# themattrosen/Planeverb

Hardware: AMD Instinct MI355X
Metric: grid_cell_updates_per_s (higher is better)
Workload: dtype f32

## Files before the change

### include/planeverb_amd.h

```cpp
#ifndef PLANEVERB_AMD_H
#define PLANEVERB_AMD_H

#include <stddef.h>
#include <stdint.h>

#ifdef __cplusplus
extern "C" {
#endif

#if defined(__GNUC__)
#define PVA_EXPORT __attribute__((visibility("default")))
#else
#define PVA_EXPORT
#endif


typedef struct PlaneverbOutput {
    float occlusion;
    float wetGain;
    float rt60;
    float lowpass;
    float directionX;
    float directionY;
    float sourceDirectionX;
// ... 78 lines not shown
    int tileRows, tileCols;
    int pitch, rows;
    int histRows, histPitch;
    int numGeometry;
    long long deviceBytes;
    int streamFuse;
    int residentKernel;
} PvAmdInfo;

typedef struct PvAmdTimings {
    float fdtdMs;
    float analysisMs;
    float geometryMs;
    float stepKernelMs;
    int stepLaunches;
    float airKernelMs;
    float generalKernelMs;
    int airLaunches, generalLaunches;
    float stepLoopMs;
    int reachedCells;
    int activeCells;
    int silentCells;
} PvAmdTimings;

enum {
    PVA_OPT_DENSE_HISTORY = 1,
    PVA_OPT_NUM_STEPS = 2,
    PVA_OPT_SKIP_ANALYSIS = 3,
    PVA_OPT_USE_GRAPH = 4,
    PVA_OPT_STEPS_PER_LAUNCH = 5,
    PVA_OPT_TILE_ROWS = 6,
    PVA_OPT_NO_FREE_GRID = 7,
    PVA_OPT_TIME_KERNELS = 8,
    PVA_OPT_TILE_ORDER = 9,
    PVA_OPT_SMALL_GRID_KERNEL = 10,
    PVA_OPT_PACKED_MATH = 11,
    PVA_OPT_STREAMING_ANALYSIS = 12,
    PVA_OPT_STREAM_ROWS = 13,
    PVA_OPT_MERGED_LAUNCH = 14,
    PVA_OPT_ROW_BANDS = 16,
    PVA_OPT_PATCH_KERNEL = 17,
    PVA_OPT_LAZY_FAR_CELLS = 19,
    PVA_OPT_STREAM_FUSE = 20,
    PVA_OPT_AUX_STREAMS = 21,
    PVA_OPT_RESIDENT_KERNEL = 22,
    PVA_OPT_RT60_LANES = 23,
    PVA_OPT_FUSED_ANALYSIS = 29,
    PVA_OPT_ANALYSIS_FORK = 28,
    PVA_OPT_STREAM_PRIORITY = 25,
    PVA_OPT_ALTERNATE_SWEEPS = 26,
    PVA_OPT_XCD_REGIONS = 27,
    PVA_OPT_REACH_BOUND = 30,
    PVA_OPT_RESIDENT_WINDOW = 31,
    PVA_OPT_DEBUG_LOSE_FIRST_CAPTURE = 24,
    PVA_OPT_PATCH_STRIP = 18,
    PVA_OPT_EDGE_TILES = 15
};

PVA_EXPORT int PvAmdDeviceCount(void);
PVA_EXPORT const char* PvAmdLastError(void);
PVA_EXPORT const char* PvAmdVersion(void);

PVA_EXPORT PvAmdSolver* PvAmdCreate(float gridSizeX, float gridSizeY, int gridResolution, int device);
PVA_EXPORT PvAmdSolver* PlaneverbCreateGrid(float gridSizeX, float gridSizeY, int gridResolution, int device);
PVA_EXPORT PvAmdSolver* PvAmdCreateSlabs(float gridSizeX, float gridSizeY, int gridResolution, const int* devices,
                                         int nslabs);
typedef struct PvAmdSlabInfo {
    int nslabs;
    int row0[16], rows[16], device[16];
    long long haloBytesPerLaunch;
    long long exchangeBytesPerRun;
    long long deviceBytes[16];
    int handoffWords;
    int streamRedeals;
    float dryRunUsPerSweep;
} PvAmdSlabInfo;
PVA_EXPORT int PvAmdGetSlabInfo(PvAmdSolver* s, PvAmdSlabInfo* out);
PVA_EXPORT PvAmdSolver* PvAmdCreateSlabRank(float gridSizeX, float gridSizeY, int gridResolution, int device,
                                            int slabIndex, int slabCount);
PVA_EXPORT int PvAmdComputeEfree(float gridSizeX, float gridSizeY, int gridResolution, int device, float* efree);
PVA_EXPORT int PvAmdSlabSetEfree(PvAmdSolver* slab, float efree);
PVA_EXPORT int PvAmdSlabBegin(PvAmdSolver* slab, float lx, float ly, float lz);
PVA_EXPORT int PvAmdSlabNumLaunches(PvAmdSolver* slab);
PVA_EXPORT int PvAmdSlabLaunch(PvAmdSolver* slab, int li);
PVA_EXPORT int PvAmdSlabHaloFloats(PvAmdSolver* slab);
PVA_EXPORT int PvAmdSlabExportHalo(PvAmdSolver* slab, int side, float* host);
PVA_EXPORT int PvAmdSlabImportHalo(PvAmdSolver* slab, int side, const float* host);
PVA_EXPORT int PvAmdSlabHistoryFloats(PvAmdSolver* slab);
PVA_EXPORT int PvAmdSlabExportEdgeHistory(PvAmdSolver* slab, float* host);
PVA_EXPORT int PvAmdSlabImportAboveHistory(PvAmdSolver* slab, const float* host);
PVA_EXPORT int PvAmdSlabAnalyze(PvAmdSolver* slab);
PVA_EXPORT long long PvAmdSlabWindowBlock(PvAmdSolver* slab, int* info4, float* host, long long capacityFloats);
typedef struct PvAmdSlabRoot PvAmdSlabRoot;
PVA_EXPORT PvAmdSlabRoot* PvAmdSlabRootCreate(PvAmdSolver* anySlab, int device);
PVA_EXPORT void PvAmdSlabRootDestroy(PvAmdSlabRoot* r);
PVA_EXPORT int PvAmdSlabRootBegin(PvAmdSlabRoot* r, float lx, float ly, float lz);
PVA_EXPORT int PvAmdSlabRootImportBlock(PvAmdSlabRoot* r, const int* info4, const float* host);
PVA_EXPORT int PvAmdSlabRootFinish(PvAmdSlabRoot* r);
PVA_EXPORT int PvAmdSlabRootGetOutput(PvAmdSlabRoot* r, float ex, float ey, float ez, PlaneverbOutput* out);
PVA_EXPORT int PvAmdSlabRootCopyResults(PvAmdSlabRoot* r, float* res8, float* delay);
PVA_EXPORT void PvAmdDestroy(PvAmdSolver* s);
PVA_EXPORT int PvAmdSetOption(PvAmdSolver* s, int key, long long value);
PVA_EXPORT int PvAmdGetInfo(PvAmdSolver* s, PvAmdInfo* out);

PVA_EXPORT int PvAmdAddGeometry(PvAmdSolver* s, float posX, float posY, float width, float height,
                                float absorption);
// ... 2 lines not shown
PVA_EXPORT int PvAmdRemoveGeometry(PvAmdSolver* s, int id);
PVA_EXPORT int PvAmdLoadScene(PvAmdSolver* s, const char* pvPath);
PVA_EXPORT int PvAmdSaveScene(PvAmdSolver* s, const char* pvPath);

PVA_EXPORT int PvAmdAddShape(PvAmdSolver* s, const float* xy, int n, float absorption);
PVA_EXPORT int PvAmdUpdateShape(PvAmdSolver* s, int id, const float* xy, int n, float absorption);
PVA_EXPORT int PvAmdRemoveShape(PvAmdSolver* s, int id);
PVA_EXPORT int PvAmdAddOrientedBox(PvAmdSolver* s, float px, float py, float w, float h, float ax, float ay, float absorption);
PVA_EXPORT int PvAmdUpdateOrientedBox(PvAmdSolver* s, int id, float px, float py, float w, float h, float ax, float ay,
                                      float absorption);
#define PVA_POLY_MAX_VERTS 64
PVA_EXPORT int PvAmdAddDisc(PvAmdSolver* s, float cx, float cy, float radius, float absorption);
PVA_EXPORT int PvAmdUpdateDisc(PvAmdSolver* s, int id, float cx, float cy, float radius, float absorption);
PVA_EXPORT int PvAmdAddCapsule(PvAmdSolver* s, float ax, float ay, float bx, float by, float radius, float absorption);
PVA_EXPORT int PvAmdUpdateCapsule(PvAmdSolver* s, int id, float ax, float ay, float bx, float by, float radius, float absorption);
PVA_EXPORT int PvAmdAddWallPath(PvAmdSolver* s, const float* xy, int n, float radius, float absorption);
PVA_EXPORT int PvAmdUpdateWallPath(PvAmdSolver* s, int id, const float* xy, int n, float radius, float absorption);
PVA_EXPORT int PvAmdAddPolygon(PvAmdSolver* s, const float* xy, int n, float absorption);
PVA_EXPORT int PvAmdUpdatePolygon(PvAmdSolver* s, int id, const float* xy, int n, float absorption);
#define PVA_MESH_SOLID 0
#define PVA_MESH_SHELL 1
#define PVA_MESH_MAX 64
#define PVA_MESH_MAX_TRIS (1 << 20)
#define PVA_MESH_MAX_TRIS_TOTAL (1 << 22)
PVA_EXPORT int PvAmdAddMesh(PvAmdSolver* s, const float* verts, int nv, const int* tris, int nt, float absorption, int mode,
                            float radius);
PVA_EXPORT int PvAmdUpdateMesh(PvAmdSolver* s, int id, const float* verts, int nv, const int* tris, int nt, float absorption,
                               int mode, float radius);
PVA_EXPORT int PvAmdSetMeshTransform(PvAmdSolver* s, int id, const float m12[12]);
PVA_EXPORT int PvAmdRemoveMesh(PvAmdSolver* s, int id);
PVA_EXPORT int PvAmdSetSliceHeight(PvAmdSolver* s, float h);
PVA_EXPORT float PvAmdGetSliceHeight(PvAmdSolver* s);
PVA_EXPORT int PvAmdMeshTriangles(PvAmdSolver* s, int id);
PVA_EXPORT int PvAmdCopyMeshSection(PvAmdSolver* s, int id, float* out4nt, uint8_t* valid_nt);
PVA_EXPORT int PvAmdHostMeshSection(const float* verts, int nv, const int* tris, int nt, const float* m12_or_null, float h,
                                    float* out4nt, uint8_t* valid_nt);
PVA_EXPORT int PvAmdHostMeshCoverage(float gridSizeX, float gridSizeY, int gridResolution, const float* verts, int nv,
                                     const int* tris, int nt, const float* m12_or_null, float h, int mode, float radius,
                                     uint8_t* cover);
PVA_EXPORT int PvAmdSetGridBoundary(PvAmdSolver* s, const float absorption4[4]);
PVA_EXPORT int PvAmdGetGridBoundary(PvAmdSolver* s, float out4[4]);
PVA_EXPORT int PvAmdSetEdgeLayer(PvAmdSolver* s, const int width4[4]);
PVA_EXPORT int PvAmdGetEdgeLayer(PvAmdSolver* s, int out4[4]);
#define PVA_EDGE_LAYER_SPLIT_R0 1e-4
PVA_EXPORT int PvAmdSetEdgeLayerSplit(PvAmdSolver* s, const int width4[4], double r0);
PVA_EXPORT int PvAmdGetEdgeLayerModel(PvAmdSolver* s, int* split, double* r0);
PVA_EXPORT int PvAmdHostEdgeLayerTables(float gridSizeX, float gridSizeY, int gridResolution, const int width4[4], float* out);
PVA_EXPORT int PvAmdHostEdgeLayerTablesR0(float gridSizeX, float gridSizeY, int gridResolution, const int width4[4], double r0,
                                          float* out);
PVA_EXPORT int PvAmdHostEnclosure(const uint8_t* beta, int nx, int ny, int seedX, int seedY, int tileRows, int tileCols, int maxTiles,
                                  int* out10);
PVA_EXPORT int PvAmdHostWindowClear(int windowRun, const int* win4, const int* prevRect4, int planesDirty, int sweptDirty,
                                    int splitPlanes);
PVA_EXPORT int PvAmdHostOrientedBoxVertices(float px, float py, float w, float h, float ax, float ay, float* out8);
PVA_EXPORT int PvAmdHostShape(const float* xy, int n, float absorption, float* out16);
PVA_EXPORT int PvAmdHostShapeCoverage(float gridSizeX, float gridSizeY, int gridResolution, const float* xy, int n,
                                      uint8_t* cover);
#define PVA_SHAPE_DISC 1
#define PVA_SHAPE_CAPSULE 2
#define PVA_SHAPE_WALL_PATH 3
#define PVA_SHAPE_POLYGON 4
PVA_EXPORT int PvAmdHostRoundShapeCoverage(float gridSizeX, float gridSizeY, int gridResolution, int kind, const float* xy,
                                           int n, float radius, uint8_t* cover);

PVA_EXPORT int PvAmdRun(PvAmdSolver* s, float lx, float ly, float lz);
PVA_EXPORT int PvAmdRunAsync(PvAmdSolver* s, float lx, float ly, float lz);
PVA_EXPORT int PvAmdRunAsyncAfter(PvAmdSolver* s, PvAmdSolver* prev, float lx, float ly, float lz);
PVA_EXPORT int PvAmdSync(PvAmdSolver* s);
PVA_EXPORT int PvAmdRunBatch(PvAmdSolver* const* solvers, int n, const float* listenersXYZ, int wait);
PVA_EXPORT float PvAmdClockProbe(int device, float* byMemtimeMHz);
PVA_EXPORT int PvAmdBandwidthProbe(int device, float* gbPerS4);
#define PVA_LIBM_LOG10               0
#define PVA_LIBM_LOG10_NONNEG        1
#define PVA_LIBM_LOG10_NONNEG_TAB    2
#define PVA_LIBM_LOG10_NORMAL_TAB    3
#define PVA_LIBM_LOG10_NORMAL_BATCH  4
#define PVA_LIBM_POW_08              5
#define PVA_LIBM_POW_23              6
#define PVA_LIBM_POW_NONNEG_08       7
#define PVA_LIBM_POW_NONNEG_23       8
#define PVA_LIBM_POW_NONNEG_TAB_08   9
#define PVA_LIBM_POW_NONNEG_TAB_23  10
PVA_EXPORT int PvAmdLibmProbe(int form, const float* in, float* out, long long n, int onDevice);
PVA_EXPORT int PvAmdGetTimings(PvAmdSolver* s, PvAmdTimings* out);
PVA_EXPORT int PvAmdLastRunResidentWindow(PvAmdSolver* s);
PVA_EXPORT int PvAmdLastRunOneXcd(PvAmdSolver* s);

PVA_EXPORT int PvAmdSetEmitters(PvAmdSolver* s, const float* xyz, int n);
PVA_EXPORT int PvAmdGetOutput(PvAmdSolver* s, float ex, float ey, float ez, PlaneverbOutput* out);
PVA_EXPORT int PvAmdSetOutputQueries(PvAmdSolver* s, const float* xyz, int n);
PVA_EXPORT int PvAmdGetQueriedOutputs(PvAmdSolver* s, PlaneverbOutput* out, int n);
#define PVA_QREC_ROOM_METRICS   1u
#define PVA_QREC_DECAY_TIMES    2u
#define PVA_QREC_LATERAL        4u
#define PVA_QREC_ECHOGRAM       8u
#define PVA_QREC_ECHO_CRITERION 16u
#define PVA_QREC_LOBES          32u
PVA_EXPORT int PvAmdSetQueryRecords(PvAmdSolver* s, unsigned kinds);
PVA_EXPORT unsigned PvAmdGetQueryRecordKinds(PvAmdSolver* s);
PVA_EXPORT int PvAmdQueryRecordFloats(PvAmdSolver* s, unsigned kind);
PVA_EXPORT int PvAmdGetQueriedRecords(PvAmdSolver* s, unsigned kind, float* out, int nQueries);
#define PVA_RECORD_QUERIES_MAX 1024
PVA_EXPORT int PvAmdSetRecordQueries(PvAmdSolver* s, const float* xyz, int n);
#define PVA_QSPEC_BAND_METRICS 1u
#define PVA_QSPEC_MODULATION   2u
#define PVA_QSPEC_SPECTRUM     4u
PVA_EXPORT int PvAmdSetQuerySpectralRecords(PvAmdSolver* s, unsigned kinds);
PVA_EXPORT unsigned PvAmdGetQuerySpectralKinds(PvAmdSolver* s);
PVA_EXPORT int PvAmdQuerySpectralFloats(PvAmdSolver* s, unsigned kind);
PVA_EXPORT int PvAmdGetQueriedSpectralRecords(PvAmdSolver* s, unsigned kind, float* out, int nQueries);
PVA_EXPORT int PvAmdSetEmitterRecords(PvAmdSolver* s, unsigned timeKinds, unsigned spectralKinds);
PVA_EXPORT int PvAmdGetEmitterRecordKinds(PvAmdSolver* s, unsigned* timeKinds, unsigned* spectralKinds);
PVA_EXPORT int PvAmdEmitterRecordFloats(PvAmdSolver* s, int family, unsigned kind);
PVA_EXPORT int PvAmdGetEmitterRecords(PvAmdSolver* s, int family, unsigned kind, float* out, int nEmitters);
PVA_EXPORT int PvAmdGetEmitterCells(PvAmdSolver* s, int* cxcy, int cap);
PVA_EXPORT int PvAmdCopyEmitterTrace(PvAmdSolver* s, int emitter, float* outT);
PVA_EXPORT int PvAmdCopyResults(PvAmdSolver* s, float* res8, float* delay);
PVA_EXPORT int PvAmdCopyResultsBlock(PvAmdSolver* s, int r0, int c0, int nr, int nc, float* res8, float* delay);
PVA_EXPORT int PvAmdGetImpulseResponse(PvAmdSolver* s, int cx, int cy, float* out3T);
PVA_EXPORT int PvAmdGetImpulseResponseCells(PvAmdSolver* s, int cx, int cy, PlaneverbCell* outT);
PVA_EXPORT int PvAmdCopyFields(PvAmdSolver* s, float* pr, float* vx, float* vy);
PVA_EXPORT int PvAmdCopyHistoryPlane(PvAmdSolver* s, int t, float* pr);
PVA_EXPORT int PvAmdSetHistoryPlane(PvAmdSolver* s, int t, const float* pr);
typedef struct PvAmdRoomMetrics {
    float c50, c80, d50, ts, e50, l50, e80, l80, total, moment;
} PvAmdRoomMetrics;
PVA_EXPORT int PvAmdComputeRoomMetrics(PvAmdSolver* s, float* ms);
PVA_EXPORT int PvAmdCopyRoomMetrics(PvAmdSolver* s, float* out10);
PVA_EXPORT int PvAmdCopyRoomMetricsBlock(PvAmdSolver* s, int r0, int c0, int nr, int nc, float* out10);
PVA_EXPORT int PvAmdGetRoomMetrics(PvAmdSolver* s, float ex, float ey, float ez, PvAmdRoomMetrics* out);
PVA_EXPORT int PvAmdHostRoomMetrics(const float* p, int T, int fs, int onset, PvAmdRoomMetrics* out);
typedef struct PvAmdDecayTimes {
    float edt, t20, t30, n_edt, n_t20, n_t30, e0, depth;
} PvAmdDecayTimes;
PVA_EXPORT int PvAmdComputeDecayTimes(PvAmdSolver* s, float* ms);
PVA_EXPORT int PvAmdCopyDecayTimes(PvAmdSolver* s, float* out8);
PVA_EXPORT int PvAmdCopyDecayTimesBlock(PvAmdSolver* s, int r0, int c0, int nr, int nc, float* out8);
PVA_EXPORT int PvAmdGetDecayTimes(PvAmdSolver* s, float ex, float ey, float ez, PvAmdDecayTimes* out);
// ... 248 lines not shown
```

### planeverb_amd/api.py

```python
import ctypes as C
import os
from collections import namedtuple

import numpy as np

from .build import LIB_PATH

PV_INVALID_DRY_GAIN = -1.0
PV_INVALID_ID = -1

PVA_OPT_DENSE_HISTORY = 1
PVA_OPT_NUM_STEPS = 2
PVA_OPT_SKIP_ANALYSIS = 3
PVA_OPT_USE_GRAPH = 4
PVA_OPT_STEPS_PER_LAUNCH = 5
PVA_OPT_TILE_ROWS = 6
PVA_OPT_NO_FREE_GRID = 7
PVA_OPT_TIME_KERNELS = 8
PVA_OPT_TILE_ORDER = 9
PVA_OPT_SMALL_GRID_KERNEL = 10
PVA_OPT_PACKED_MATH = 11
PVA_OPT_STREAMING_ANALYSIS = 12
PVA_OPT_STREAM_ROWS = 13
PVA_OPT_MERGED_LAUNCH = 14
PVA_OPT_EDGE_TILES = 15
PVA_OPT_ROW_BANDS = 16
PVA_OPT_PATCH_KERNEL = 17
PVA_OPT_PATCH_STRIP = 18
PVA_OPT_LAZY_FAR_CELLS = 19
PVA_OPT_STREAM_FUSE = 20
PVA_OPT_AUX_STREAMS = 21
PVA_OPT_RESIDENT_KERNEL = 22
PVA_OPT_RT60_LANES = 23
PVA_OPT_DEBUG_LOSE_FIRST_CAPTURE = 24
PVA_OPT_STREAM_PRIORITY = 25
PVA_OPT_ALTERNATE_SWEEPS = 26
PVA_OPT_XCD_REGIONS = 27
PVA_OPT_ANALYSIS_FORK = 28
PVA_OPT_FUSED_ANALYSIS = 29
PVA_OPT_REACH_BOUND = 30
PVA_OPT_RESIDENT_WINDOW = 31


class PlaneverbOutput(C.Structure):
    _fields_ = [("occlusion", C.c_float), ("wetGain", C.c_float), ("rt60", C.c_float), ("lowpass", C.c_float),
                ("directionX", C.c_float), ("directionY", C.c_float), ("sourceDirectionX", C.c_float),
                ("sourceDirectionY", C.c_float)]

    def as_array(self):
        return np.array([self.occlusion, self.wetGain, self.rt60, self.lowpass, self.directionX, self.directionY,
                         self.sourceDirectionX, self.sourceDirectionY], np.float32)


class PlaneverbCell(C.Structure):
    _fields_ = [("pr", C.c_float), ("vx", C.c_float), ("vy", C.c_float), ("b", C.c_short), ("by", C.c_short)]


CELL_DTYPE = np.dtype([("pr", np.float32), ("vx", np.float32), ("vy", np.float32), ("b", np.int16), ("by", np.int16)])


class PvAmdInfo(C.Structure):
    _fields_ = [("gx", C.c_int), ("gy", C.c_int), ("T", C.c_int), ("fs", C.c_int), ("res", C.c_int),
                ("dx", C.c_float), ("dt", C.c_float), ("efree", C.c_float), ("device", C.c_int),
                ("stepsPerLaunch", C.c_int), ("tileRows", C.c_int), ("tileCols", C.c_int), ("pitch", C.c_int),
                ("rows", C.c_int), ("histRows", C.c_int), ("histPitch", C.c_int), ("numGeometry", C.c_int),
                ("deviceBytes", C.c_longlong), ("streamFuse", C.c_int), ("residentKernel", C.c_int)]


class PvAmdBakeInfo(C.Structure):
    _fields_ = [("gx", C.c_int), ("gy", C.c_int), ("T", C.c_int), ("fs", C.c_int), ("res", C.c_int), ("dx", C.c_float),
                ("stride", C.c_int), ("x0", C.c_float), ("z0", C.c_float), ("sx", C.c_float), ("sz", C.c_float),
                ("nx", C.c_int), ("nz", C.c_int), ("probesBaked", C.c_int), ("probesInvalid", C.c_int),
                ("records", C.c_longlong), ("materialHash", C.c_ulonglong)]


class PvAmdSlabInfo(C.Structure):
    _fields_ = [("nslabs", C.c_int), ("row0", C.c_int * 16), ("rows", C.c_int * 16), ("device", C.c_int * 16),
                ("haloBytesPerLaunch", C.c_longlong), ("exchangeBytesPerRun", C.c_longlong),
                ("deviceBytes", C.c_longlong * 16), ("handoffWords", C.c_int), ("streamRedeals", C.c_int),
                ("dryRunUsPerSweep", C.c_float)]


class PvAmdTimings(C.Structure):
    _fields_ = [("fdtdMs", C.c_float), ("analysisMs", C.c_float), ("geometryMs", C.c_float),
                ("stepKernelMs", C.c_float), ("stepLaunches", C.c_int), ("airKernelMs", C.c_float), ("generalKernelMs", C.c_float), ("airLaunches", C.c_int),
                ("generalLaunches", C.c_int), ("stepLoopMs", C.c_float), ("reachedCells", C.c_int), ("activeCells", C.c_int), ("silentCells", C.c_int)]


ROOM_METRIC_NAMES = ("c50", "c80", "d50", "ts", "e50", "l50", "e80", "l80", "total", "moment")


class PvAmdRoomMetrics(C.Structure):
    _fields_ = [(n, C.c_float) for n in ROOM_METRIC_NAMES]

# ... 116 lines not shown
    "PvAmdUpdateGeometry": (C.c_int, [_vp, C.c_int] + [C.c_float] * 5),
    "PvAmdRemoveGeometry": (C.c_int, [_vp, C.c_int]),
    "PvAmdLoadScene": (C.c_int, [_vp, C.c_char_p]),
    "PvAmdSaveScene": (C.c_int, [_vp, C.c_char_p]),
    "PvAmdAddShape": (C.c_int, [_vp, _fp, C.c_int, C.c_float]),
    "PvAmdUpdateShape": (C.c_int, [_vp, C.c_int, _fp, C.c_int, C.c_float]),
    "PvAmdRemoveShape": (C.c_int, [_vp, C.c_int]),
    "PvAmdAddOrientedBox": (C.c_int, [_vp] + [C.c_float] * 7),
    "PvAmdUpdateOrientedBox": (C.c_int, [_vp, C.c_int] + [C.c_float] * 7),
    "PvAmdAddDisc": (C.c_int, [_vp] + [C.c_float] * 4),
    "PvAmdUpdateDisc": (C.c_int, [_vp, C.c_int] + [C.c_float] * 4),
    "PvAmdAddCapsule": (C.c_int, [_vp] + [C.c_float] * 6),
    "PvAmdUpdateCapsule": (C.c_int, [_vp, C.c_int] + [C.c_float] * 6),
    "PvAmdAddWallPath": (C.c_int, [_vp, _fp, C.c_int, C.c_float, C.c_float]),
    "PvAmdUpdateWallPath": (C.c_int, [_vp, C.c_int, _fp, C.c_int, C.c_float, C.c_float]),
    "PvAmdAddPolygon": (C.c_int, [_vp, _fp, C.c_int, C.c_float]),
    "PvAmdUpdatePolygon": (C.c_int, [_vp, C.c_int, _fp, C.c_int, C.c_float]),
    "PvAmdAddMesh": (C.c_int, [_vp, _fp, C.c_int, C.POINTER(C.c_int), C.c_int, C.c_float, C.c_int, C.c_float]),
    "PvAmdUpdateMesh": (C.c_int, [_vp, C.c_int, _fp, C.c_int, C.POINTER(C.c_int), C.c_int, C.c_float, C.c_int, C.c_float]),
    "PvAmdSetMeshTransform": (C.c_int, [_vp, C.c_int, _fp]),
    "PvAmdRemoveMesh": (C.c_int, [_vp, C.c_int]),
    "PvAmdSetSliceHeight": (C.c_int, [_vp, C.c_float]),
    "PvAmdGetSliceHeight": (C.c_float, [_vp]),
    "PvAmdMeshTriangles": (C.c_int, [_vp, C.c_int]),
    "PvAmdCopyMeshSection": (C.c_int, [_vp, C.c_int, _fp, C.POINTER(C.c_ubyte)]),
    "PvAmdHostMeshSection": (C.c_int, [_fp, C.c_int, C.POINTER(C.c_int), C.c_int, _fp, C.c_float, _fp, C.POINTER(C.c_ubyte)]),
    "PvAmdHostMeshCoverage": (C.c_int, [C.c_float, C.c_float, C.c_int, _fp, C.c_int, C.POINTER(C.c_int), C.c_int, _fp, C.c_float,
                                        C.c_int, C.c_float, C.POINTER(C.c_ubyte)]),
    "PvAmdSetGridBoundary": (C.c_int, [_vp, _fp]),
    "PvAmdGetGridBoundary": (C.c_int, [_vp, _fp]),
    "PlaneverbSetGridBoundary": (None, [C.c_float] * 4),
    "PvAmdSetEdgeLayer": (C.c_int, [_vp, C.POINTER(C.c_int)]),
    "PvAmdGetEdgeLayer": (C.c_int, [_vp, C.POINTER(C.c_int)]),
    "PlaneverbSetEdgeLayer": (None, [C.c_int] * 4),
    "PvAmdSetEdgeLayerSplit": (C.c_int, [_vp, C.POINTER(C.c_int), C.c_double]),
    "PvAmdGetEdgeLayerModel": (C.c_int, [_vp, C.POINTER(C.c_int), C.POINTER(C.c_double)]),
    "PlaneverbSetEdgeLayerSplit": (None, [C.c_int] * 4),
    "PvAmdHostEdgeLayerTablesR0": (C.c_int, [C.c_float, C.c_float, C.c_int, C.POINTER(C.c_int), C.c_double, _fp]),
    "PvAmdHostEdgeLayerTables": (C.c_int, [C.c_float, C.c_float, C.c_int, C.POINTER(C.c_int), _fp]),
    "PvAmdHostEnclosure": (C.c_int, [C.POINTER(C.c_ubyte)] + [C.c_int] * 7 + [C.POINTER(C.c_int)]),
    "PvAmdHostOrientedBoxVertices": (C.c_int, [C.c_float] * 6 + [_fp]),
    "PvAmdHostShape": (C.c_int, [_fp, C.c_int, C.c_float, _fp]),
    "PvAmdHostShapeCoverage": (C.c_int, [C.c_float, C.c_float, C.c_int, _fp, C.c_int, C.POINTER(C.c_ubyte)]),
    "PvAmdHostRoundShapeCoverage": (C.c_int, [C.c_float, C.c_float, C.c_int, C.c_int, _fp, C.c_int, C.c_float,
                                              C.POINTER(C.c_ubyte)]),
    "PvAmdRun": (C.c_int, [_vp] + [C.c_float] * 3),
    "PvAmdRunAsync": (C.c_int, [_vp] + [C.c_float] * 3),
    "PvAmdRunAsyncAfter": (C.c_int, [_vp, _vp] + [C.c_float] * 3),
    "PvAmdSync": (C.c_int, [_vp]),
    "PvAmdRunBatch": (C.c_int, [C.POINTER(_vp), C.c_int, _fp, C.c_int]),
    "PvAmdGetTimings": (C.c_int, [_vp, C.POINTER(PvAmdTimings)]),
    "PvAmdLastRunResidentWindow": (C.c_int, [_vp]),
    "PvAmdLastRunOneXcd": (C.c_int, [_vp]),
    "PvAmdHostWindowClear": (C.c_int, [C.c_int, C.POINTER(C.c_int), C.POINTER(C.c_int), C.c_int, C.c_int, C.c_int]),
    "PvAmdClockProbe": (C.c_float, [C.c_int, _fp]),
    "PvAmdBandwidthProbe": (C.c_int, [C.c_int, _fp]),
    "PvAmdSetEmitters": (C.c_int, [_vp, _fp, C.c_int]),
    "PvAmdGetOutput": (C.c_int, [_vp] + [C.c_float] * 3 + [C.POINTER(PlaneverbOutput)]),
    "PvAmdSetOutputQueries": (C.c_int, [_vp, _fp, C.c_int]),
    "PvAmdGetQueriedOutputs": (C.c_int, [_vp, C.POINTER(PlaneverbOutput), C.c_int]),
    "PvAmdSetQueryRecords": (C.c_int, [_vp, C.c_uint]),
    "PvAmdGetQueryRecordKinds": (C.c_uint, [_vp]),
    "PvAmdQueryRecordFloats": (C.c_int, [_vp, C.c_uint]),
    "PvAmdGetQueriedRecords": (C.c_int, [_vp, C.c_uint, _fp, C.c_int]),
    "PvAmdSetRecordQueries": (C.c_int, [_vp, _fp, C.c_int]),
    "PvAmdSetQuerySpectralRecords": (C.c_int, [_vp, C.c_uint]),
    "PvAmdGetQuerySpectralKinds": (C.c_uint, [_vp]),
    "PvAmdQuerySpectralFloats": (C.c_int, [_vp, C.c_uint]),
    "PvAmdGetQueriedSpectralRecords": (C.c_int, [_vp, C.c_uint, _fp, C.c_int]),
    "PvAmdSetEmitterRecords": (C.c_int, [_vp, C.c_uint, C.c_uint]),
    "PvAmdGetEmitterRecordKinds": (C.c_int, [_vp, C.POINTER(C.c_uint), C.POINTER(C.c_uint)]),
    "PvAmdEmitterRecordFloats": (C.c_int, [_vp, C.c_int, C.c_uint]),
    "PvAmdGetEmitterRecords": (C.c_int, [_vp, C.c_int, C.c_uint, _fp, C.c_int]),
    "PvAmdGetEmitterCells": (C.c_int, [_vp, C.POINTER(C.c_int), C.c_int]),
    "PvAmdCopyEmitterTrace": (C.c_int, [_vp, C.c_int, _fp]),
    "PvAmdCopyResults": (C.c_int, [_vp, _fp, _fp]),
    "PvAmdCopyResultsBlock": (C.c_int, [_vp, C.c_int, C.c_int, C.c_int, C.c_int, _fp, _fp]),
    "PvAmdGetImpulseResponse": (C.c_int, [_vp, C.c_int, C.c_int, _fp]),
    "PvAmdGetImpulseResponseCells": (C.c_int, [_vp, C.c_int, C.c_int, C.POINTER(PlaneverbCell)]),
    "PvAmdCopyFields": (C.c_int, [_vp, _fp, _fp, _fp]),
    "PvAmdCopyHistoryPlane": (C.c_int, [_vp, C.c_int, _fp]),
    "PvAmdSetHistoryPlane": (C.c_int, [_vp, C.c_int, _fp]),
    "PvAmdLibmProbe": (C.c_int, [C.c_int, _fp, _fp, C.c_longlong, C.c_int]),
    "PvAmdComputeRoomMetrics": (C.c_int, [_vp, _fp]),
    "PvAmdCopyRoomMetrics": (C.c_int, [_vp, _fp]),
    "PvAmdCopyRoomMetricsBlock": (C.c_int, [_vp, C.c_int, C.c_int, C.c_int, C.c_int, _fp]),
    "PvAmdGetRoomMetrics": (C.c_int, [_vp] + [C.c_float] * 3 + [C.POINTER(PvAmdRoomMetrics)]),
    "PvAmdHostRoomMetrics": (C.c_int, [_fp, C.c_int, C.c_int, C.c_int, C.POINTER(PvAmdRoomMetrics)]),
    "PvAmdComputeDecayTimes": (C.c_int, [_vp, _fp]),
    "PvAmdCopyDecayTimes": (C.c_int, [_vp, _fp]),
    "PvAmdCopyDecayTimesBlock": (C.c_int, [_vp, C.c_int, C.c_int, C.c_int, C.c_int, _fp]),
    "PvAmdGetDecayTimes": (C.c_int, [_vp] + [C.c_float] * 3 + [C.POINTER(PvAmdDecayTimes)]),
    "PvAmdHostDecayTimes": (C.c_int, [_fp, C.c_int, C.c_int, C.c_int, C.POINTER(PvAmdDecayTimes)]),
    "PvAmdComputeEchoCriterion": (C.c_int, [_vp, _fp]),
    "PvAmdCopyEchoCriterion": (C.c_int, [_vp, _fp]),
    "PvAmdCopyEchoCriterionBlock": (C.c_int, [_vp, C.c_int, C.c_int, C.c_int, C.c_int, _fp]),
    "PvAmdGetEchoCriterion": (C.c_int, [_vp] + [C.c_float] * 3 + [C.POINTER(PvAmdEchoCriterion)]),
    "PvAmdHostEchoCriterion": (C.c_int, [_fp, C.c_int, C.c_int, C.c_int, C.POINTER(PvAmdEchoCriterion)]),
    "PvAmdComputeLateralFraction": (C.c_int, [_vp, _fp]),
    "PvAmdCopyLateralFraction": (C.c_int, [_vp, _fp]),
    "PvAmdCopyLateralFractionBlock": (C.c_int, [_vp, C.c_int, C.c_int, C.c_int, C.c_int, _fp]),
    "PvAmdGetLateralFraction": (C.c_int, [_vp] + [C.c_float] * 3 + [C.POINTER(PvAmdLateralFraction)]),
    "PvAmdHostLateralFraction": (C.c_int, [_fp, _fp, _fp, C.c_int, C.c_int, C.c_int, C.POINTER(PvAmdLateralFraction)]),
    "PvAmdSetEchogram": (C.c_int, [_vp, C.c_float, C.c_int]),
    "PvAmdGetEchogramSlots": (C.c_int, [_vp, _fp, C.POINTER(C.c_int)]),
    "PvAmdComputeEchogram": (C.c_int, [_vp, _fp]),
# ... 501 lines not shown
    a, n = _xy(vertices)
    cover = np.empty((i.gx + 1, i.gy + 1), np.uint8)
    _check(lib().PvAmdHostShapeCoverage(float(size_x), float(size_y), int(res), _f(a), n,
                                        cover.ctypes.data_as(C.POINTER(C.c_ubyte))))
    return cover


EDGE_LAYER_DEFAULT_WIDTH = 24
EDGE_LAYER_SPLIT_R0 = 1e-4


def _w4(w4):
    a = np.ascontiguousarray(w4, np.int32).reshape(-1)
    if a.size != 4:
        raise ValueError("four widths: x = 0, x = gx, y = 0, y = gy")
    return a


def edge_layer_tables(size_x, size_y, res, w4, r0=None):
    i = host_grid_info(size_x, size_y, res)
    a = _w4(w4)
    out = np.empty(4 * (i.gx + 1) + 4 * (i.gy + 1), np.float32)
    wp = a.ctypes.data_as(C.POINTER(C.c_int))
    if r0 is None:
        n = lib().PvAmdHostEdgeLayerTables(float(size_x), float(size_y), int(res), wp, _f(out))
    else:
        n = lib().PvAmdHostEdgeLayerTablesR0(float(size_x), float(size_y), int(res), wp, float(r0), _f(out))
    if n < 0:
        raise PlaneverbError(last_error())
    nx, ny = i.gx + 1, i.gy + 1
    names = ["apx", "bpx", "ax", "bx", "apy", "bpy", "ay", "by"]
    offs = [0, nx, 2 * nx, 3 * nx, 4 * nx, 4 * nx + ny, 4 * nx + 2 * ny, 4 * nx + 3 * ny]
    return {k: out[o:o + (nx if j < 4 else ny)].copy() for j, (k, o) in enumerate(zip(names, offs))}


def host_enclosure(beta, seed, tile_rows=36, tile_cols=40, max_tiles=128):
    b = np.ascontiguousarray(beta, np.uint8)
    out = np.zeros(10, np.int32)
    if lib().PvAmdHostEnclosure(b.ctypes.data_as(C.POINTER(C.c_ubyte)), b.shape[0], b.shape[1], int(seed[0]), int(seed[1]),
                                int(tile_rows), int(tile_cols), int(max_tiles), out.ctypes.data_as(C.POINTER(C.c_int))) < 0:
        raise PlaneverbError(last_error())
    v = [int(x) for x in out]
    return dict(found=v[0], cells=v[1], box=tuple(v[2:6]), window=tuple(v[6:10]))


def host_window_clear(window_run, win, prev_rect, planes_dirty, swept_dirty, split_planes):
    w, p = ((C.c_int * 4)(*[int(v) for v in r]) for r in (win, prev_rect))
    rc = lib().PvAmdHostWindowClear(int(bool(window_run)), w, p, int(bool(planes_dirty)), int(bool(swept_dirty)), int(bool(split_planes)))
    if rc < 0:
        raise PlaneverbError(last_error())
    return rc


def load_pv(path, max_boxes=4096):
    buf = np.empty((max_boxes, 5), np.float32)
    n = lib().PvAmdHostLoadPv(path.encode(), _f(buf), max_boxes)
    if n < 0:
        raise PlaneverbError(last_error())
    return buf[:n].copy()


def save_pv(path, boxes, ids=None):
    b = np.ascontiguousarray(boxes, np.float32).reshape(-1, 5)
    ida = None if ids is None else np.ascontiguousarray(ids, np.int32)
    _check(lib().PvAmdHostSavePv(path.encode(), _f(b), None if ida is None else ida.ctypes.data_as(C.POINTER(C.c_int)),
                                 len(b)))


def host_room_metrics(p, fs, onset):
    a = np.ascontiguousarray(p, np.float32).reshape(-1)
    out = PvAmdRoomMetrics()
    _check(lib().PvAmdHostRoomMetrics(_f(a) if a.size else None, int(a.size), int(fs), int(onset), out))
    return out.as_array()


def host_decay_times(p, fs, onset):
    a = np.ascontiguousarray(p, np.float32).reshape(-1)
    out = PvAmdDecayTimes()
    _check(lib().PvAmdHostDecayTimes(_f(a) if a.size else None, int(a.size), int(fs), int(onset), out))
    return out.as_array()


def host_echo_criterion(p, fs, onset):
    a = np.ascontiguousarray(p, np.float32).reshape(-1)
    out = PvAmdEchoCriterion()
    _check(lib().PvAmdHostEchoCriterion(_f(a) if a.size else None, int(a.size), int(fs), int(onset), out))
    return out.as_array()


def host_lateral_fraction(p, vx, vy, fs, onset):
    a, x, y = (np.ascontiguousarray(v, np.float32).reshape(-1) for v in (p, vx, vy))
    if not (a.size == x.size == y.size):
        raise ValueError("host_lateral_fraction: p, vx and vy must have the same length")
    out = PvAmdLateralFraction()
    ptr = [_f(v) if v.size else None for v in (a, x, y)]
    _check(lib().PvAmdHostLateralFraction(ptr[0], ptr[1], ptr[2], int(a.size), int(fs), int(onset), out))
    return out.as_array()


ECHOGRAM_MAX_SLOTS = 32


def host_echogram(p, vx, vy, fs, onset, slot_seconds, n_slots):
    a, x, y = (np.ascontiguousarray(v, np.float32).reshape(-1) for v in (p, vx, vy))
    if not (a.size == x.size == y.size):
        raise ValueError("host_echogram: p, vx and vy must have the same length")
# ... 682 lines not shown
    def import_block(self, info4, data):
        info = (C.c_int * 4)(*[int(v) for v in info4])
        data = np.ascontiguousarray(data, np.float32)
        _check(lib().PvAmdSlabRootImportBlock(self._h, info, _f(data) if data.size else None))

    def finish(self):
        _check(lib().PvAmdSlabRootFinish(self._h))

    def get_output(self, emitter):
        o = PlaneverbOutput()
        _check(lib().PvAmdSlabRootGetOutput(self._h, *[float(v) for v in emitter], o))
        return o

    def results(self):
        res = np.empty((self.gx, self.gy, 8), np.float32)
        delay = np.empty((self.gx, self.gy), np.float32)
        _check(lib().PvAmdSlabRootCopyResults(self._h, _f(res), _f(delay)))
        return res, delay


def run_batch(solvers, listeners, wait=True):
    n = len(solvers)
    if n != len(listeners):
        raise ValueError("one listener position per solver")
    hs = (_vp * n)(*[sv._h for sv in solvers])
    xyz = (C.c_float * (3 * n))(*[float(v) for L in listeners for v in L])
    _check(lib().PvAmdRunBatch(hs, n, xyz, 1 if wait else 0))


class Solver:

    def __init__(self, size_x, size_y, res, device=0, slabs=None, **options):
        if slabs is not None:
            dev = (C.c_int * len(slabs))(*[int(d) for d in slabs])
            self._h = lib().PvAmdCreateSlabs(float(size_x), float(size_y), int(res), dev, len(slabs))
        else:
            self._h = lib().PvAmdCreate(float(size_x), float(size_y), int(res), int(device))
        if not self._h:
            raise PlaneverbError(last_error())
        keys = {"dense_history": PVA_OPT_DENSE_HISTORY, "num_steps": PVA_OPT_NUM_STEPS,
                "skip_analysis": PVA_OPT_SKIP_ANALYSIS, "use_graph": PVA_OPT_USE_GRAPH,
                "steps_per_launch": PVA_OPT_STEPS_PER_LAUNCH, "tile_rows": PVA_OPT_TILE_ROWS,
                "no_free_grid": PVA_OPT_NO_FREE_GRID, "time_kernels": PVA_OPT_TIME_KERNELS,
                "tile_order": PVA_OPT_TILE_ORDER, "small_grid_kernel": PVA_OPT_SMALL_GRID_KERNEL,
                "packed_math": PVA_OPT_PACKED_MATH, "streaming_analysis": PVA_OPT_STREAMING_ANALYSIS,
                "stream_rows": PVA_OPT_STREAM_ROWS, "merged_launch": PVA_OPT_MERGED_LAUNCH,
                "edge_tiles": PVA_OPT_EDGE_TILES, "row_bands": PVA_OPT_ROW_BANDS,
                "patch_kernel": PVA_OPT_PATCH_KERNEL, "patch_strip": PVA_OPT_PATCH_STRIP,
                "lazy_far_cells": PVA_OPT_LAZY_FAR_CELLS, "stream_fuse": PVA_OPT_STREAM_FUSE, "aux_streams": PVA_OPT_AUX_STREAMS,
                "resident_kernel": PVA_OPT_RESIDENT_KERNEL, "rt60_lanes": PVA_OPT_RT60_LANES,
                "debug_lose_first_capture": PVA_OPT_DEBUG_LOSE_FIRST_CAPTURE, "stream_priority": PVA_OPT_STREAM_PRIORITY,
                "alternate_sweeps": PVA_OPT_ALTERNATE_SWEEPS, "xcd_regions": PVA_OPT_XCD_REGIONS,
                "analysis_fork": PVA_OPT_ANALYSIS_FORK, "fused_analysis": PVA_OPT_FUSED_ANALYSIS,
                "reach_bound": PVA_OPT_REACH_BOUND, "resident_window": PVA_OPT_RESIDENT_WINDOW}
        for k, v in options.items():
            _check(lib().PvAmdSetOption(self._h, keys[k], int(v)))
        self.info = PvAmdInfo()
        _check(lib().PvAmdGetInfo(self._h, self.info))
        i = self.info
        self.gx, self.gy, self.T, self.fs, self.dx, self.dt, self.efree = i.gx, i.gy, i.T, i.fs, i.dx, i.dt, i.efree
        self._pulse_len = host_grid_info(size_x, size_y, res).T

    def close(self):
        if getattr(self, "_h", None):
            lib().PvAmdDestroy(self._h)
            self._h = None

    def __del__(self):
        try:
            self.close()
        except Exception:
            pass

    def __enter__(self):
        return self

    def __exit__(self, *a):
        self.close()

    def slab_info(self):
        i = PvAmdSlabInfo()
        _check(lib().PvAmdGetSlabInfo(self._h, i))
        return i

    def load_scene(self, path):
        n = lib().PvAmdLoadScene(self._h, path.encode())
        if n < 0:
            raise PlaneverbError(last_error())
        return n

    def save_scene(self, path):
        _check(lib().PvAmdSaveScene(self._h, path.encode()))

    def add_geometry(self, aabb):
        return lib().PvAmdAddGeometry(self._h, *[float(v) for v in aabb])

    def update_geometry(self, gid, aabb):
        _check(lib().PvAmdUpdateGeometry(self._h, int(gid), *[float(v) for v in aabb]))

    def remove_geometry(self, gid):
        _check(lib().PvAmdRemoveGeometry(self._h, int(gid)))

    def add_shape(self, vertices, absorption):
        a, n = _xy(vertices)
        sid = lib().PvAmdAddShape(self._h, _f(a), n, float(absorption))
        if sid < 0:
            raise PlaneverbError(last_error())
# ... 85 lines not shown
        return seg, valid

    def set_grid_boundary(self, r4):
        a = np.ascontiguousarray(r4, np.float32).reshape(-1)
        if a.size != 4:
            raise ValueError("four absorption values: x = 0, x = gx, y = 0, y = gy")
        _check(lib().PvAmdSetGridBoundary(self._h, _f(a)))

    def grid_boundary(self):
        out = np.zeros(4, np.float32)
        _check(lib().PvAmdGetGridBoundary(self._h, _f(out)))
        return out

    def set_edge_layer(self, w4):
        a = _w4(w4)
        _check(lib().PvAmdSetEdgeLayer(self._h, a.ctypes.data_as(C.POINTER(C.c_int))))
        _check(lib().PvAmdGetInfo(self._h, self.info))

    def edge_layer(self):
        out = np.zeros(4, np.int32)
        _check(lib().PvAmdGetEdgeLayer(self._h, out.ctypes.data_as(C.POINTER(C.c_int))))
        return out

    def set_edge_layer_split(self, w4, r0=EDGE_LAYER_SPLIT_R0):
        a = _w4(w4)
        _check(lib().PvAmdSetEdgeLayerSplit(self._h, a.ctypes.data_as(C.POINTER(C.c_int)), float(r0)))
        _check(lib().PvAmdGetInfo(self._h, self.info))

    def edge_layer_model(self):
        sp, r0 = C.c_int(0), C.c_double(0.0)
        _check(lib().PvAmdGetEdgeLayerModel(self._h, C.byref(sp), C.byref(r0)))
        return ("split" if sp.value else "unsplit"), r0.value

    def run(self, listener):
        _check(lib().PvAmdRun(self._h, *[float(v) for v in listener]))

    def run_async(self, listener):
        _check(lib().PvAmdRunAsync(self._h, *[float(v) for v in listener]))

    def run_async_after(self, prev, listener):
        _check(lib().PvAmdRunAsyncAfter(self._h, prev._h, *[float(v) for v in listener]))

    def sync(self):
        _check(lib().PvAmdSync(self._h))

    def run_steps(self, nsteps, with_pulse=False, listener=(0.0, 0.0, 0.0)):
        _check(lib().PvAmdRunSteps(self._h, int(nsteps), int(with_pulse), float(listener[0]), float(listener[2])))

    def last_run_resident_window(self):
        rc = lib().PvAmdLastRunResidentWindow(self._h)
        if rc < 0:
            raise PlaneverbError(last_error())
        return rc == 1

    def last_run_one_xcd(self):
        rc = lib().PvAmdLastRunOneXcd(self._h)
        if rc < 0:
            raise PlaneverbError(last_error())
        return rc == 1

    def timings(self):
        t = PvAmdTimings()
        _check(lib().PvAmdGetTimings(self._h, t))
        return t

    def set_emitters(self, emitters):
        e = np.ascontiguousarray(emitters, np.float32).reshape(-1, 3)
        _check(lib().PvAmdSetEmitters(self._h, _f(e), len(e)))

    def get_output(self, emitter):
        o = PlaneverbOutput()
        _check(lib().PvAmdGetOutput(self._h, *[float(v) for v in emitter], o))
        return o

    def set_output_queries(self, emitters):
        e = np.ascontiguousarray(np.asarray(emitters, np.float32).reshape(-1, 3))
        self._nq = len(e)
        _check(lib().PvAmdSetOutputQueries(self._h, _f(e), len(e)))

    def queried_outputs(self):
        n = getattr(self, "_nq", 0)
        out = (PlaneverbOutput * max(n, 1))()
        _check(lib().PvAmdGetQueriedOutputs(self._h, out, n))
        return np.frombuffer(out, np.float32).reshape(-1, 8)[:n].copy()

    def set_query_records(self, kinds):
        _check(lib().PvAmdSetQueryRecords(self._h, int(kinds)))

    def _record_floats(self, floats, kind):
        n = floats(self._h, int(kind))
        if n < 0:
            raise PlaneverbError(last_error())
        return n

    def _read_records(self, read, kind, shape):
        n = getattr(self, "_nrq", 0) or getattr(self, "_nq", 0)
        out = np.empty((n,) + shape, np.float32)
        _check(read(self._h, int(kind), _f(out) if n else None, n))
        return out

    def query_record_kinds(self):
        return int(lib().PvAmdGetQueryRecordKinds(self._h))

    def query_record_floats(self, kind):
        return self._record_floats(lib().PvAmdQueryRecordFloats, kind)

# ... 570 lines not shown
```

### planeverb_amd/csrc/pv_analysis.h

```cpp
#pragma once

#include <hip/hip_runtime.h>

#include <cfloat>

#include "pv_device.h"
#include "pv_prims.h"

namespace pva {

__device__ __forceinline__ bool analysisAborted(const AnalyzeArgs& a) { return a.abortWord && *a.abortWord != 0u; }

struct NearBox {
    int r0, c0, r1, c1;
    __device__ __forceinline__ bool holds(int r, int c) const { return r >= r0 && r <= r1 && c >= c0 && c <= c1; }
};
__device__ __forceinline__ NearBox nearBoxOf(const int* box, int wr0, int wc0, int wnr, int wnc) {
    NearBox b;
    b.r0 = max(box[0] - 1, wr0);
    b.c0 = max(box[1] - 1, wc0);
    b.r1 = min(box[2] + 1, wr0 + wnr - 1);
    b.c1 = min(box[3] + 1, wc0 + wnc - 1);
    return b;
}
__device__ __forceinline__ NearBox nearBoxOf(const AnalyzeArgs& a, const DynParams& dyn) {
    const int wr0 = dyn.histRow0 - a.G, wc0 = dyn.histCol0 - a.G;
    return nearBoxOf(a.box, wr0, wc0, min(a.winRows, a.gx - wr0), min(a.winCols, a.gy - wc0));
}

__device__ __forceinline__ void farDirectionOf(const FarInfo& f, long long cell, float* ox, float* oy) {
    const int r = (int)(cell / f.gy), c = (int)(cell - (long long)r * f.gy);
    float x = (float)r * f.dx - f.lx, y = (float)c * f.dx - f.lz;
    float len = (x * x) + (y * y);
    if (len != 0.f) {
        len = sqrtf(len);
        x /= len;
        y /= len;
    }
    *ox = x;
    *oy = y;
}
__device__ __forceinline__ bool isFarCell(const FarInfo& f, long long cell) {
    if (!f.on) return false;
    const int r = (int)(cell / f.gy), c = (int)(cell - (long long)r * f.gy);
    if (f.box) return !nearBoxOf(f.box, f.r0, f.c0, f.nr, f.nc).holds(r, c);
    return r < f.r0 || r >= f.r0 + f.nr || c < f.c0 || c >= f.c0 + f.nc;
}

struct CellHistory {
    const float* h;
    long long plane;
    __device__ __forceinline__ float at(int t) const { return h[(long long)t * plane]; }
};

struct PlaneCell {
    bool inGrid;
    int X, Y;
    int tile;
    int row, col;
    int g;
    int hti, htj;
};
__device__ __forceinline__ PlaneCell planeCell(const AnalyzeArgs& a, const DynParams& dyn, long long g) {
    PlaneCell c{false, 0, 0, 0, 0, 0, 0, 0, 0};
// ... 79 lines not shown
```

### planeverb_amd/csrc/pv_analysis.hip

```cpp
#include <hip/hip_runtime.h>

#include <cfloat>
#include <climits>
#include <cstdint>

#include "pv_analysis.h"
#include "pv_analysis_dev.h"
#include "pv_device.h"
#include "pv_launch.h"
#include "pv_libm.h"
#include "pv_prims.h"
#include "pv_record_lane.h"
#include "pv_zone_maps.h"

namespace pva {



template <int CH>
__device__ __forceinline__ void rt60Chunk(const float (&pc)[CH], const int i0, const int startingPoint, float& edc,
                                          float& xysum, float& ysum) {
    float e[CH], y[CH];
#pragma unroll
    for (int k = 0; k < CH; ++k) {
        edc = (i0 - k >= startingPoint) ? edc + pc[k] * pc[k] : edc;
        e[k] = edc;
    }
#pragma unroll
    for (int k = 0; k < CH; ++k) y[k] = 10.f * pvLog10fNonNeg(e[k]);
#pragma unroll
    for (int k = 0; k < CH; ++k) {
        const bool v = i0 - k >= startingPoint;
        xysum = v ? xysum + y[k] * (float)(i0 - k - startingPoint) : xysum;
        ysum = v ? ysum + y[k] : ysum;
    }
}

__device__ __forceinline__ bool analysisWindowCell(const AnalyzeArgs& a, const DynParams& dyn, int* X, int* Y) {
    const int wc = blockIdx.x * blockDim.x + threadIdx.x, wr = blockIdx.y;
    if (wc >= a.winCols) return false;
    *X = dyn.histRow0 - a.G + wr;
    *Y = dyn.histCol0 - a.G + wc;
    return *X < a.gx && *Y < a.gy;
}

#ifndef PV_ONSET_WAVES
#define PV_ONSET_WAVES 4
#endif
#ifndef PV_ONSET_SC
#define PV_ONSET_SC 32
#endif
constexpr int kOnsetWaves = PV_ONSET_WAVES, kOnsetSC = PV_ONSET_SC;
__global__ __launch_bounds__(64 * kOnsetWaves) void pv_onset_kernel(const AnalyzeArgs a) {
    __shared__ int found[64];
    if (analysisAborted(a)) return;
    const DynParams dyn = *a.dyn;
    const int lane = threadIdx.x & 63, wave = __builtin_amdgcn_readfirstlane((int)(threadIdx.x >> 6));
    const long long g = (long long)blockIdx.x * 64 + lane;
    const PlaneCell c = planeCell(a, dyn, g);
    const int T = a.T;
    int tF = INT_MAX;
    bool live = c.inGrid;
    if (live) {
        tF = a.tileFirst[c.tile];
        live = tF < T && a.coef[(size_t)(c.X + a.G) * a.pitch + (c.Y + a.G)].beta != 0.f;
    }
    const bool air = live;
    if (a.labels) {
        const int lX = dyn.lrow - a.G, lY = dyn.lcol - a.G;
        const int mine = live ? a.labels[(size_t)c.X * a.labelNY + c.Y] : -1;
        const int theirs = (lX >= 0 && lX <= a.gx && lY >= 0 && lY < a.labelNY) ? a.labels[(size_t)lX * a.labelNY + lY] : -2;
        live = live && mine == theirs;
    }
    if (wave == 0) found[lane] = INT_MAX;
    if (a.stamp && blockIdx.x == 0 && threadIdx.x == 0) a.stamp[1] = wall_clock64();
    __syncthreads();
    bool inPrev = false;
    if (a.box) {
        const int p0 = a.prevBox[0], p1 = a.prevBox[1], p2 = min(a.prevBox[2], a.gx - 1), p3 = min(a.prevBox[3], a.gy - 1);
        inPrev = c.inGrid && c.X >= p0 && c.X <= p2 && c.Y >= p1 && c.Y <= p3;
        if (p2 >= p0 && p3 >= p1) {
            const int wr0 = dyn.histRow0 - a.G, wc0 = dyn.histCol0 - a.G;
            const int wr1 = wr0 + min(a.winRows, a.gx - wr0) - 1, wc1 = wc0 + min(a.winCols, a.gy - wc0) - 1;
            if (p0 < wr0 || p2 > wr1 || p1 < wc0 || p3 > wc1)
                for (int r = p0 + (int)blockIdx.x; r <= p2; r += (int)gridDim.x)
                    for (int cc = p1 + (int)threadIdx.x; cc <= p3; cc += (int)blockDim.x)
                        if (r < wr0 || r > wr1 || cc < wc0 || cc > wc1) a.delay[r * a.gy + cc] = FLT_MAX;
        }
    }
    if (a.wholeWindow || a.box) {
        if (wave == 0 && c.inGrid && !live && (a.wholeWindow || inPrev)) a.delay[c.X * a.gy + c.Y] = FLT_MAX;
        if (blockIdx.x == 0 && wave == 1) {
            int n = 0;
            for (int i = lane; i < dyn.histTilesX * dyn.histTilesY; i += 64) {
                const int ti = dyn.histTileX0 + i / dyn.histTilesY, tj = dyn.histTileY0 + i % dyn.histTilesY;
                if (a.tileFirst[ti * a.nty + tj] < T) n += a.rxi * a.wi;
            }
#pragma unroll
            for (int off = 1; off < 64; off <<= 1) n += __shfl_xor(n, off);
            if (lane == 0) a.activeCount[0] = n;
        }
    }
    if (__ballot(live) == 0ull) {
        const unsigned long long ms = __ballot(air);
        if (wave == 0 && lane == 0 && ms) atomicAdd(a.activeCount + 3, __popcll(ms));
        return;
    }
    const int m = abs(c.X - (dyn.lrow - a.G)) + abs(c.Y - (dyn.lcol - a.G));
    const int tS = live ? min(max(tF, m), T) : INT_MAX;
    int tBeg = tS;
#pragma unroll
    for (int off = 1; off < 64; off <<= 1) tBeg = min(tBeg, __shfl_xor(tBeg, off));
    tBeg = __builtin_amdgcn_readfirstlane(tBeg);
    const int voff = (int)g * 4;
    const int planeBytes = (int)(a.histPlane * 4);
    constexpr int SC = kOnsetSC;
#pragma unroll 1
    for (int t = tBeg + wave * SC; t < T; t += kOnsetWaves * SC) {
        const int best = found[lane];
        if (__ballot(live && best > t) == 0ull) break;
        float pc[SC];
#pragma unroll
        for (int k = 0; k < SC; ++k) {
            const int tt = t + k;
            const bool want = live && tt >= tS && tt < T && tt < best;
            pc[k] = bufLoadF(makeRsrc(a.hist + (long long)min(tt, T - 1) * a.histPlane, planeBytes), want ? voff : 0x7fffffff, 0);
        }
        int hit = INT_MAX;
#pragma unroll
        for (int k = SC - 1; k >= 0; --k) hit = fabsf(pc[k]) > kAudibleThresholdDev ? t + k : hit;
        if (hit != INT_MAX) atomicMin(&found[lane], hit);
    }
    __syncthreads();
    if (wave != 0) return;
    const int onset = found[lane];
    if (live) {
        if (onset != INT_MAX) a.delay[c.X * a.gy + c.Y] = (float)onset;
        else if (a.wholeWindow || inPrev) a.delay[c.X * a.gy + c.Y] = FLT_MAX;
    }
    const bool reached = live && onset != INT_MAX;
    const unsigned long long mr = __ballot(reached), ms = __ballot(air && !reached);
    if (a.box && mr) {
        int r0 = reached ? c.X : INT_MAX, c0 = reached ? c.Y : INT_MAX, r1 = reached ? c.X : -1, c1 = reached ? c.Y : -1;
#pragma unroll
        for (int off = 1; off < 64; off <<= 1) {
            r0 = min(r0, __shfl_xor(r0, off));
            c0 = min(c0, __shfl_xor(c0, off));
            r1 = max(r1, __shfl_xor(r1, off));
            c1 = max(c1, __shfl_xor(c1, off));
        }
        if (lane == 0) {
            const int b0 = __hip_atomic_load(a.box + 0, __ATOMIC_RELAXED, __HIP_MEMORY_SCOPE_AGENT);
            const int b1 = __hip_atomic_load(a.box + 1, __ATOMIC_RELAXED, __HIP_MEMORY_SCOPE_AGENT);
            const int b2 = __hip_atomic_load(a.box + 2, __ATOMIC_RELAXED, __HIP_MEMORY_SCOPE_AGENT);
            const int b3 = __hip_atomic_load(a.box + 3, __ATOMIC_RELAXED, __HIP_MEMORY_SCOPE_AGENT);
            if (r0 < b0) atomicMin(a.box + 0, r0);
            if (c0 < b1) atomicMin(a.box + 1, c0);
            if (r1 > b2) atomicMax(a.box + 2, r1);
            if (c1 > b3) atomicMax(a.box + 3, c1);
        }
    }
    if (lane == 0) {
        if (mr) {
            atomicAdd(a.activeCount + 1, __popcll(mr));
            a.unitList[atomicAdd(a.activeCount + 4, 1)] = (int)blockIdx.x;
        }
        if (ms) atomicAdd(a.activeCount + 3, __popcll(ms));
    }
}

__global__ __launch_bounds__(256) void pv_encode_kernel(const AnalyzeArgs a) {
    if (analysisAborted(a)) return;
    const DynParams dyn = *a.dyn;
    const int unit = blockIdx.x * 4 + (int)(threadIdx.x >> 6);
    if (unit >= a.activeCount[4]) return;
    const PlaneCell pc0 = planeCell(a, dyn, (long long)a.unitList[unit] * 64 + (threadIdx.x & 63));
    const float delay = pc0.inGrid ? a.delay[pc0.X * a.gy + pc0.Y] : FLT_MAX;
    const bool live = delay != FLT_MAX;
    if (__ballot(live) == 0ull) return;
    encodeWave<false>(a, dyn, pc0, live, live ? (int)delay : 0, rt60LanesPerCell(a, a.activeCount[1]) == 1);
}

template <int L>
__global__ __launch_bounds__(256) void pv_encode_groups_kernel(const AnalyzeArgs a) {
    if (analysisAborted(a)) return;
    const DynParams dyn = *a.dyn;
    constexpr int BPU = L / 4;
    const int unit = blockIdx.x / BPU;
    if (unit >= a.activeCount[4]) return;
    const int ww = (blockIdx.x % BPU) * 4 + (int)(threadIdx.x >> 6), lane = threadIdx.x & 63;
    const PlaneCell pc0 = planeCell(a, dyn, (long long)a.unitList[unit] * 64 + ww * (64 / L) + lane / L);
    const float delay = pc0.inGrid ? a.delay[pc0.X * a.gy + pc0.Y] : FLT_MAX;
    const bool live = delay != FLT_MAX;
    if (__ballot(live) == 0ull) return;
    encodeGroups<L, false>(a, dyn, pc0, lane % L, live, live ? (int)delay : 0);
}

__device__ __forceinline__ void countActiveCells(const AnalyzeArgs& a) {
    __shared__ int part[256];
    const DynParams dyn = *a.dyn;
    int n = 0;
    for (int i = threadIdx.x; i < dyn.histTilesX * dyn.histTilesY; i += 256) {
        const int ti = dyn.histTileX0 + i / dyn.histTilesY, tj = dyn.histTileY0 + i % dyn.histTilesY;
        if (a.tileFirst[ti * a.nty + tj] < a.T) n += a.rxi * a.wi;
    }
    part[threadIdx.x] = n;
    __syncthreads();
    for (int w = 128; w > 0; w >>= 1) {
        if ((int)threadIdx.x < w) part[threadIdx.x] += part[threadIdx.x + w];
        __syncthreads();
    }
    if (threadIdx.x == 0) {
        a.activeCount[0] = part[0];
        a.activeCount[1] = 0;
        a.activeCount[3] = 0;
        a.activeCount[4] = 0;
    }
}
// ... 59 lines not shown
    const float thresholdDist = 0.3f * wavelength;

    while (delay > kDelayCloseDev && loudness < kDistanceGainDev) {
        const int r = cur / a.gy, c = cur - r * a.gy;
        float bestLoud = 0.f, bestDelay = FLT_MAX;
        for (int i = 0; i < 8; ++i) {
            const int nr = r + neighbourDr(i), nc = c + neighbourDc(i);
            if (nr < 0 || nc < 0 || nr >= a.gx || nc >= a.gy) continue;
            const int ni = nr * a.gy + nc;
            const float occ = a.out[ni];
            const float d = a.delay[ni];
            if (occ == 0.f) continue;
            if (d < bestDelay && occ > 0.f) {
                bestLoud = occ;
                cur = ni;
                bestDelay = d;
            }
        }
        if (bestDelay == FLT_MAX || bestDelay >= delay) break;
        delay = bestDelay;
        loudness = bestLoud;
        const float geodesic = kCDev * bestDelay / samplingRate;
        const int r2 = cur / a.gy, c2 = cur - r2 * a.gy;
        const float tx = (float)r2 * a.dx - a.lx, ty = (float)c2 * a.dx - a.lz;
        const float euclid = sqrtf((tx * tx) + (ty * ty));
        if (fabsf(geodesic - euclid) < thresholdDist) break;
    }
    storeDirection(a, index, cur);
}
__global__ __launch_bounds__(256) void pv_direction_kernel(const AnalyzeArgs a) {
    if (analysisAborted(a)) return;
    const DynParams dyn = *a.dyn;
    forDirectionCells(a, dyn, [&](const int index) { directionWalkCell(a, index); });
}

__global__ __launch_bounds__(256) void pv_dir_init_kernel(const AnalyzeArgs a, int* J) {
    if (analysisAborted(a)) return;
    const DynParams dyn = *a.dyn;
    forDirectionCells(a, dyn, [&](const int p) { dirInitCell<false>(a, dyn, J, p); });
}

__global__ __launch_bounds__(256) void pv_dir_jump_kernel(const AnalyzeArgs a, int* J) {
    if (analysisAborted(a)) return;
    const DynParams dyn = *a.dyn;
    forDirectionCells(a, dyn, [&](const int p) { dirJumpCell<false>(a, dyn, J, p); });
}

__global__ __launch_bounds__(256) void pv_dir_final_kernel(const AnalyzeArgs a, const int* J) {
    if (analysisAborted(a)) return;
    const DynParams dyn = *a.dyn;
    forDirectionCells(a, dyn, [&](const int p) { dirFinalCell<false>(a, dyn, J, p); });
}

static dim3 analysisWindowGrid(const AnalyzeArgs& a) { return dim3((a.winCols + 255) / 256, a.winRows); }

static void launchDirectionJump(const AnalyzeArgs& a, int* J, hipStream_t stream) {
    const dim3 grid = analysisWindowGrid(a), block(256);
    hipLaunchKernelGGL(pv_dir_init_kernel, grid, block, 0, stream, a, J);
    for (int i = 0; i < dirJumpPasses(a.T); ++i) hipLaunchKernelGGL(pv_dir_jump_kernel, grid, block, 0, stream, a, J);
    hipLaunchKernelGGL(pv_dir_final_kernel, grid, block, 0, stream, a, J);
}

__global__ void pv_fill_delay_kernel(float* delay, int n) {
    const int i = blockIdx.x * blockDim.x + threadIdx.x;
    if (i < n) delay[i] = FLT_MAX;
}

void launchFarCells(const AnalyzeArgs& a, hipStream_t stream) {
    const int n = a.gx * a.gy;
    hipLaunchKernelGGL(pv_far_cells_kernel, dim3((n + 255) / 256), dim3(256), 0, stream, a);
}

void launchOnset(const AnalyzeArgs& a, hipStream_t stream) {
    hipLaunchKernelGGL(pv_onset_kernel, dim3((unsigned)((a.histPlane + 63) / 64)), dim3(64 * kOnsetWaves), 0, stream, a);
}
void launchEncode(const AnalyzeArgs& a, hipStream_t stream) {
    const unsigned units = (unsigned)((a.histPlane + 63) / 64);
    if (a.rt60Lanes != 1 && a.histPlane <= 16384)
        hipLaunchKernelGGL(pv_encode_groups_kernel<16>, dim3(units * 4), dim3(256), 0, stream, a);
    else if (a.rt60Lanes != 1 && a.histPlane <= kRt60TileMinCells)
        hipLaunchKernelGGL(pv_encode_groups_kernel<4>, dim3(units), dim3(256), 0, stream, a);
    else
        hipLaunchKernelGGL(pv_encode_kernel, dim3((unsigned)((a.histPlane + 255) / 256)), dim3(256), 0, stream, a);
}
void launchRt60(const AnalyzeArgs& a, hipStream_t stream) { launchRt60Forms(a, stream); }

void launchAnalysisCells(const AnalyzeArgs& a, hipStream_t stream) {
    launchOnset(a, stream);
    launchEncode(a, stream);
    launchRt60(a, stream);
}

void launchAnalysisDirection(const AnalyzeArgs& a, hipStream_t stream) {
    const dim3 grid = analysisWindowGrid(a);
    if (a.dirJump)
        launchDirectionJump(a, a.dirScratch, stream);
    else
        hipLaunchKernelGGL(pv_direction_kernel, grid, dim3(256), 0, stream, a);
}

void launchFillDelay(float* delay, long long n, hipStream_t stream) {
    hipLaunchKernelGGL(pv_fill_delay_kernel, dim3((unsigned)((n + 255) / 256)), dim3(256), 0, stream, delay, (int)n);
}

void launchAnalysisFar(const AnalyzeArgs& a, hipStream_t stream) {
    if (a.wholeWindow || a.box) return;
    const int n = a.gx * a.gy;
    if (a.lazyFar) {
        const int nr = max(a.prevNR, min(a.winRows, a.gx)), nc = max(a.prevNC, min(a.winCols, a.gy));
        hipLaunchKernelGGL(pv_far_frame_kernel, dim3((unsigned)((max(nc, 1) + 255) / 256), (unsigned)max(nr, 1), 2), dim3(256), 0,
                           stream, a);
    } else {
        hipLaunchKernelGGL(pv_far_cells_kernel, dim3((n + 255) / 256), dim3(256), 0, stream, a);
    }
}

void launchAnalysis(const AnalyzeArgs& a, hipStream_t stream) {
    launchAnalysisFar(a, stream);
    launchAnalysisCells(a, stream);
    launchAnalysisDirection(a, stream);
}


__global__ __launch_bounds__(256) void pv_stream_accum_kernel(const AnalyzeArgs a) {
    int X, Y;
    if (a.ringList) {
        const int chunks = (a.rxi * a.wi + 255) / 256;
        const int entry = blockIdx.x / chunks;
        const int t = a.ringList[entry];
        const int idx = (blockIdx.x - entry * chunks) * blockDim.x + threadIdx.x;
        if (idx >= a.rxi * a.wi) return;
        const int ti = t / a.nty, r = idx / a.wi;
        X = ti * a.rxi + r;
        Y = (t - ti * a.nty) * a.wi + (idx - r * a.wi);
    } else {
        Y = blockIdx.x * blockDim.x + threadIdx.x;
// ... 227 lines not shown
```

### planeverb_amd/csrc/pv_capi.cpp

```cpp
#include <algorithm>
#include <climits>
#include <cmath>
#include <cstdio>
#include <cstring>
#include <memory>
#include <new>
#include <string>

#include "../../include/planeverb_amd.h"
#include "pv_context.h"
#include "pv_core.h"
#include "pv_bands.h"
#include "pv_modulation.h"
#include "pv_decay.h"
#include "pv_echo.h"
#include "pv_echogram.h"
#include "pv_lateral.h"
#include "pv_lobes.h"
#include "pv_metrics.h"
#include "pv_query_records.h"
#include "pv_query_spectral.h"
#include "pv_spectrum.h"
#include "pv_waterfall.h"
#include "pv_arrays.h"
// ... 640 lines not shown
    std::memset(out, 0, sizeof(*out));
    if (valid)
        std::memcpy(out, v, sizeof(*out));
    else
        out->occlusion = kInvalidDryGain;
    return 0;
} PV_API_CATCH(-1)
int PvAmdSlabRootCopyResults(PvAmdSlabRoot* h, float* res8, float* delay) try {
    return (h && h->r) ? rootRet(h, h->r->copyResults(res8, delay)) : -1;
} PV_API_CATCH(-1)

void PvAmdDestroy(PvAmdSolver* h) try {
    delete h;
} PV_API_CATCH_VOID

int PvAmdSetOption(PvAmdSolver* h, int key, long long value) try {
    if (!h) return -1;
    if (h->s || h->g) {
        g_lastError = "options must be set before the solver is first used";
        return -1;
    }
    switch (key) {
        case PVA_OPT_DENSE_HISTORY: h->opt.denseHistory = value != 0; break;
        case PVA_OPT_NUM_STEPS: h->opt.numSteps = (int)value; break;
        case PVA_OPT_SKIP_ANALYSIS: h->opt.skipAnalysis = value != 0; break;
        case PVA_OPT_USE_GRAPH: h->opt.useGraph = (int)value; break;
        case PVA_OPT_STEPS_PER_LAUNCH: h->opt.K = (int)value; break;
        case PVA_OPT_TILE_ROWS: h->opt.rxi = (int)value; break;
        case PVA_OPT_NO_FREE_GRID: h->opt.withFreeGrid = value == 0; break;
        case PVA_OPT_TIME_KERNELS: h->opt.timeKernels = (int)value; break;
        case PVA_OPT_TILE_ORDER: h->opt.tileOrder = (int)value; break;
        case PVA_OPT_SMALL_GRID_KERNEL: h->opt.smallGrid = (int)value; break;
        case PVA_OPT_PACKED_MATH: h->opt.packed = value != 0; break;
        case PVA_OPT_STREAMING_ANALYSIS: h->opt.streaming = value != 0; break;
        case PVA_OPT_STREAM_ROWS: h->opt.segments = (int)value; break;
        case PVA_OPT_MERGED_LAUNCH: h->opt.merged = (int)value; break;
        case PVA_OPT_EDGE_TILES: h->opt.edgeTiles = value != 0; break;
        case PVA_OPT_ROW_BANDS: h->opt.rowBands = (int)value; break;
        case PVA_OPT_PATCH_KERNEL: h->opt.patch = (int)value; break;
        case PVA_OPT_LAZY_FAR_CELLS: h->opt.lazyFar = value != 0; break;
        case PVA_OPT_STREAM_FUSE: h->opt.streamFuse = (int)value; break;
        case PVA_OPT_AUX_STREAMS: h->opt.auxStreams = (int)std::max<long long>(0, std::min<long long>(value, 8)); break;
        case PVA_OPT_PATCH_STRIP: h->opt.patchStrip = (int)value; break;
        case PVA_OPT_RESIDENT_KERNEL: h->opt.resident = (int)value; break;
        case PVA_OPT_RT60_LANES: h->opt.rt60Lanes = (int)value; break;
        case PVA_OPT_ANALYSIS_FORK: h->opt.analysisFork = (int)value; break;
        case PVA_OPT_FUSED_ANALYSIS: h->opt.fusedAnalysis = (int)value; break;
        case PVA_OPT_DEBUG_LOSE_FIRST_CAPTURE: h->opt.debugLoseFirstCapture = value != 0; break;
        case PVA_OPT_STREAM_PRIORITY: h->opt.streamPriority = (int)value; break;
        case PVA_OPT_ALTERNATE_SWEEPS: h->opt.alternateSweeps = (int)value; break;
        case PVA_OPT_XCD_REGIONS: h->opt.xcdRegions = (int)value; break;
        case PVA_OPT_REACH_BOUND: h->opt.reachBound = (int)value; break;
        case PVA_OPT_RESIDENT_WINDOW: h->opt.residentWindow = (int)value; break;
        default: g_lastError = "unknown option"; return -1;
    }
    return 0;
} PV_API_CATCH(-1)

int PvAmdGetInfo(PvAmdSolver* h, PvAmdInfo* out) try {
    if (!out || !ensure(h, true)) return -1;
    if (h->g) {
        const GridSpec& g = h->g->spec();
        const Solver* s0 = h->g->slab(0);
        std::memset(out, 0, sizeof(*out));
        out->gx = g.gx;
        out->gy = g.gy;
        out->T = h->g->T();
        out->fs = (int)g.fs;
        out->res = g.res;
        out->dx = g.dx;
        out->dt = g.dt;
        out->efree = h->g->efree();
        out->device = s0->device();
        out->stepsPerLaunch = s0->K();
        out->tileRows = s0->geometry().rxi;
        out->tileCols = s0->geometry().wi;
        out->pitch = s0->geometry().pitch;
        out->rows = s0->geometry().rows;
        out->histRows = s0->histRows();
        out->histPitch = s0->histPitch();
        out->numGeometry = h->g->numBoxes();
        out->deviceBytes = h->g->deviceBytes();
        return 0;
    }
    const GridSpec& g = h->s->spec();
    const Geometry& geo = h->s->geometry();
    std::memset(out, 0, sizeof(*out));
    out->gx = g.gx;
    out->gy = g.gy;
    out->T = h->s->T();
    out->fs = (int)g.fs;
    out->res = g.res;
    out->dx = g.dx;
    out->dt = g.dt;
    out->efree = h->s->efree();
    out->device = h->s->device();
    out->stepsPerLaunch = h->s->K();
    out->tileRows = geo.rxi;
    out->tileCols = geo.wi;
    out->pitch = geo.pitch;
    out->rows = geo.rows;
    out->histRows = h->s->histRows();
    out->histPitch = h->s->histPitch();
    out->numGeometry = h->s->numBoxes();
    out->deviceBytes = h->s->deviceBytes();
    out->streamFuse = h->s->streamFuse() ? 1 : 0;
// ... 306 lines not shown
    Solver* s[kBatchMax];
    for (int i = 0; i < n; ++i) {
        if (!wholeGrid(hs[i]) || !ensure(hs[i])) return -1;
        s[i] = hs[i]->s;
    }
    std::string err;
    if (Solver::runBatch(s, n, listenersXYZ, wait != 0, &err)) return 0;
    g_lastError = err.empty() ? "batched run failed" : err;
    return -1;
} PV_API_CATCH(-1)

int PvAmdSync(PvAmdSolver* h) try {
    if (!wholeGrid(h) || !ensure(h)) return -1;
    return ret(h, h->s->sync());
} PV_API_CATCH(-1)

float PvAmdClockProbe(int device, float* byMemtimeMHz) try {
    return clockProbeMHz(device, byMemtimeMHz);
} PV_API_CATCH(0.f)

int PvAmdBandwidthProbe(int device, float* gbPerS4) try {
    if (!gbPerS4) return -1;
    if (bandwidthProbeGBs(device, gbPerS4)) return 0;
    g_lastError = "PvAmdBandwidthProbe: allocation or launch failed (2 GiB of device memory are needed)";
    return -1;
} PV_API_CATCH(-1)

int PvAmdLibmProbe(int form, const float* in, float* out, long long n, int onDevice) try {
    return libmProbe(form, in, out, n, onDevice != 0, &g_lastError) ? 0 : -1;
} PV_API_CATCH(-1)

int PvAmdGetTimings(PvAmdSolver* h, PvAmdTimings* out) try {
    if (!out || !ensure(h, true)) return -1;
    const SolverTimings& t = h->g ? h->g->timings() : h->s->timings();
    out->fdtdMs = t.fdtdMs;
    out->analysisMs = t.analysisMs;
    out->geometryMs = t.geometryMs;
    out->stepLaunches = t.stepLaunches;
    out->stepKernelMs = t.stepLaunches ? t.fdtdMs / (float)t.stepLaunches : 0.f;
    out->airKernelMs = t.airKernelMs;
    out->generalKernelMs = t.generalKernelMs;
    out->airLaunches = t.airLaunches;
    out->generalLaunches = t.generalLaunches;
    out->stepLoopMs = t.stepLoopMs;
    out->reachedCells = t.reachedCells;
    out->activeCells = t.activeCells;
    out->silentCells = t.silentCells;
    return 0;
} PV_API_CATCH(-1)

int PvAmdLastRunResidentWindow(PvAmdSolver* h) try {
    if (!wholeGrid(h) || !ensure(h, true)) return -1;
    return h->s->lastRunResidentWindow() ? 1 : 0;
} PV_API_CATCH(-1)

int PvAmdLastRunOneXcd(PvAmdSolver* h) try {
    if (!wholeGrid(h) || !ensure(h, true)) return -1;
    return h->s->lastRunOneXcd() ? 1 : 0;
} PV_API_CATCH(-1)

int PvAmdSetEmitters(PvAmdSolver* h, const float* xyz, int n) try {
    if (!wholeGrid(h) || !ensure(h) || (n > 0 && !xyz)) return -1;
    return ret(h, h->s->setEmitters(xyz, n));
} PV_API_CATCH(-1)

int PvAmdGetOutput(PvAmdSolver* h, float ex, float ey, float ez, PlaneverbOutput* out) try {
    if (!wholeGrid(h) || !out || !ensure(h, true)) return -1;
    float v[8];
    bool valid = false;
    if (!(h->g ? h->g->getOutput(ex, ey, ez, v, &valid) : h->s->getOutput(ex, ey, ez, v, &valid))) return ret(h, false);
    if (!valid) {
        std::memset(out, 0, sizeof(*out));
        out->occlusion = kInvalidDryGain;
        return 0;
    }
    std::memcpy(out, v, sizeof(*out));
    return 0;
} PV_API_CATCH(-1)

int PvAmdSetOutputQueries(PvAmdSolver* h, const float* xyz, int n) try {
    if (!wholeGrid(h) || (n > 0 && !xyz) || !ensure(h)) return -1;
    return ret(h, h->s->setOutputQueries(xyz, n));
} PV_API_CATCH(-1)

int PvAmdGetQueriedOutputs(PvAmdSolver* h, PlaneverbOutput* out, int n) try {
    if (n < 0 || n > Solver::kMaxQueries || (n > 0 && !out) || !wholeGrid(h) || !ensure(h)) return -1;
    float v[Solver::kMaxQueries * 8];
    unsigned char valid[Solver::kMaxQueries];
    if (!h->s->queriedOutputs(v, valid, n)) return ret(h, false);
    for (int i = 0; i < n; ++i) {
        if (valid[i]) {
            std::memcpy(&out[i], v + 8 * i, sizeof(PlaneverbOutput));
        } else {
            std::memset(&out[i], 0, sizeof(PlaneverbOutput));
            out[i].occlusion = kInvalidDryGain;
        }
    }
    return 0;
} PV_API_CATCH(-1)

static bool analysisHandle(PvAmdSolver* h, const char* pre);
static bool analysisCall(PvAmdSolver* h, const char* pre, const char* fn, const void* out);
static const char kQrecPre[] = "query records: ", kQspecPre[] = "spectral records: ";
static_assert(PVA_QSPEC_BAND_METRICS == 1u << kQspecBandMetrics && PVA_QSPEC_MODULATION == 1u << kQspecModulation &&
                  PVA_QSPEC_SPECTRUM == 1u << kQspecSpectrum,
              "planeverb_amd.h vs pv_query_spectral.h");
// ... 999 lines not shown
} PV_API_CATCH(-1)

static int hostEdgeLayerTables(float sx, float sy, int res, const int* width4, double r0, float* out, const char* name) {
    if (res < kLowResolution || !width4 || !out) {
        g_lastError = std::string(name) + ": resolution below 275 or a null array";
        return -1;
    }
    if (!edgeLayerR0Ok(r0)) {
        g_lastError = std::string(name) + ": r0 must lie strictly between 0 and 1";
        return -1;
    }
    const GridSpec g = makeGridSpec(sx, sy, res);
    if (g.gx < 1 || g.gy < 1) {
        g_lastError = std::string(name) + ": grid has no cells";
        return -1;
    }
    const char* why = edgeLayerRefusal(g.gx, g.gy, width4);
    if (*why) {
        g_lastError = std::string(name) + ": " + why;
        return -1;
    }
    edgeLayerTables(g.gx, g.gy, g.courant, width4, out, r0);
    return 4 * (g.NX + g.NY);
}

int PvAmdHostEdgeLayerTables(float sx, float sy, int res, const int* width4, float* out) try {
    return hostEdgeLayerTables(sx, sy, res, width4, kEdgeLayerR0, out, "PvAmdHostEdgeLayerTables");
} PV_API_CATCH(-1)

int PvAmdHostEdgeLayerTablesR0(float sx, float sy, int res, const int* width4, double r0, float* out) try {
    return hostEdgeLayerTables(sx, sy, res, width4, r0, out, "PvAmdHostEdgeLayerTablesR0");
} PV_API_CATCH(-1)

int PvAmdHostEnclosure(const uint8_t* beta, int nx, int ny, int seedX, int seedY, int tileRows, int tileCols, int maxTiles,
                       int* out10) try {
    if (!beta || !out10 || nx < 1 || ny < 1 || tileRows < 1 || tileCols < 1 || (long long)nx * ny > INT_MAX) {
        g_lastError = "PvAmdHostEnclosure: bad arguments";
        return -1;
    }
    const Enclosure e = findEnclosure(beta, nx, ny, seedX, seedY, tileRows, tileCols, maxTiles, nullptr);
    const int v[10] = {e.found, e.cells, e.r0, e.c0, e.r1, e.c1, e.ti0, e.tj0, e.tis, e.tjs};
    std::copy(v, v + 10, out10);
    return e.cells;
} PV_API_CATCH(-1)

int PvAmdHostWindowClear(int windowRun, const int* win4, const int* prevRect4, int planesDirty, int sweptDirty, int splitPlanes) try {
    if (!win4 || !prevRect4) {
        g_lastError = "PvAmdHostWindowClear: bad arguments";
        return -1;
    }
    return (int)planClear(windowRun != 0, win4, prevRect4, planesDirty != 0, sweptDirty != 0, splitPlanes != 0);
} PV_API_CATCH(-1)

int PvAmdHostLoadPv(const char* path, float* b5, int maxBoxes) try {
    if (!path) return -1;
    std::vector<Box> boxes;
    if (!loadPv(path, &boxes, &g_lastError)) return -1;
    for (int i = 0; i < (int)boxes.size() && i < maxBoxes; ++i) {
        b5[5 * i] = boxes[(size_t)i].x;
        b5[5 * i + 1] = boxes[(size_t)i].y;
        b5[5 * i + 2] = boxes[(size_t)i].w;
        b5[5 * i + 3] = boxes[(size_t)i].h;
        b5[5 * i + 4] = boxes[(size_t)i].R;
    }
    return (int)boxes.size();
} PV_API_CATCH(-1)

int PvAmdHostSavePv(const char* path, const float* b5, const int* ids, int n) try {
    if (!path || (n > 0 && !b5)) return -1;
    std::vector<std::pair<int, Box>> boxes;
    for (int i = 0; i < n; ++i)
        boxes.emplace_back(ids ? ids[i] : i, Box{b5[5 * i], b5[5 * i + 1], b5[5 * i + 2], b5[5 * i + 3], b5[5 * i + 4]});
    return savePv(path, boxes, &g_lastError) ? 0 : -1;
} PV_API_CATCH(-1)

int PvAmdHostRoomMetrics(const float* p, int T, int fs, int onset, PvAmdRoomMetrics* out) try {
    if (!p || !out || T <= 0 || onset < 0 || onset >= T) {
        g_lastError = "PvAmdHostRoomMetrics: an impulse response p[T], T > 0, 0 <= onset < T and an output record";
        return -1;
    }
    static_assert(sizeof(PvAmdRoomMetrics) == kRoomMetricFloats * sizeof(float), "ten floats");
    float v[kRoomMetricFloats];
    roomMetricsOfIr(p, T, fs, onset, v);
    std::memcpy(out, v, sizeof(*out));
    return 0;
} PV_API_CATCH(-1)

int PvAmdHostDecayTimes(const float* p, int T, int fs, int onset, PvAmdDecayTimes* out) try {
    if (!p || !out || T <= 0 || onset < 0 || onset >= T) {
        g_lastError = "decay times: PvAmdHostDecayTimes: an impulse response p[T], T > 0, 0 <= onset < T and an output record";
        return -1;
    }
    static_assert(sizeof(PvAmdDecayTimes) == kDecayFloats * sizeof(float), "eight floats");
    float v[kDecayFloats];
    decayTimesOfIr(p, T, fs, onset, v);
    std::memcpy(out, v, sizeof(*out));
    return 0;
} PV_API_CATCH(-1)

int PvAmdHostLateralFraction(const float* p, const float* vx, const float* vy, int T, int fs, int onset,
                             PvAmdLateralFraction* out) try {
    if (!p || !vx || !vy || !out || T <= 0 || onset < 0 || onset >= T) {
        g_lastError = "lateral fraction: PvAmdHostLateralFraction: an impulse response p[T], vx[T], vy[T], T > 0, 0 <= onset < T and an output record";
        return -1;
    }
    static_assert(sizeof(PvAmdLateralFraction) == kLateralFloats * sizeof(float), "eleven floats");
// ... 517 lines not shown
```

### planeverb_amd/csrc/pv_core.cpp

```cpp
#include "pv_core.h"

#include <cstdio>
#include <cstring>

#include <algorithm>
#include <cmath>
#include <fstream>
#include <iomanip>
#include <limits>
#include <sstream>

namespace pva {

static void fillDerived(GridSpec& g) {
    const float irSeconds = kSqrt2 * 12.5f / kC + 0.25f;
    g.T = (int)(unsigned)((float)g.fs * irSeconds);
    g.courant = kC * g.dt / g.dx;
    g.nDir = (int)(kDryDirectionLen * (float)g.fs);
    g.nDry = (int)(kDryGainLen * (float)g.fs);
    g.nWet = (int)(kWetGainLen * (float)g.fs);
    g.nCut = (int)(kSchroederOffset * (float)g.fs);
    g.nFree = g.nDry + (int)((1.f / kC) * (float)(int)g.fs);
    g.NX = g.gx + 1;
    g.NY = g.gy + 1;
// ... 687 lines not shown
    bool fits = true;
    auto window = [&]() {
        const int lo = std::max(e.r0 - 1, 0), hi = std::min(e.r1 + 1, NX - 1);
        const int lc = std::max(e.c0 - 1, 0), hc = std::min(e.c1 + 1, NY - 1);
        e.ti0 = lo / rxi;
        e.tis = hi / rxi - e.ti0 + 1;
        e.tj0 = lc / wi;
        e.tjs = hc / wi - e.tj0 + 1;
        return (long long)e.tis * e.tjs <= maxTiles;
    };
    for (size_t head = 0; head < todo.size() && fits; ++head) {
        const int i = todo[head], x = i / NY, y = i - x * NY;
        if (x < e.r0 || x > e.r1 || y < e.c0 || y > e.c1) {
            e.r0 = std::min(e.r0, x);
            e.r1 = std::max(e.r1, x);
            e.c0 = std::min(e.c0, y);
            e.c1 = std::max(e.c1, y);
            fits = window();
        }
        if (!fits) break;
        const int nb[4] = {x > 0 ? i - NY : -1, x + 1 < NX ? i + NY : -1, y > 0 ? i - 1 : -1, y + 1 < NY ? i + 1 : -1};
        for (int j : nb)
            if (j >= 0 && beta[(size_t)j] && mark(j)) {
                if ((long long)todo.size() >= cap) {
                    fits = false;
                    break;
                }
                todo.push_back(j);
            }
    }
    e.cells = (int)todo.size();
    for (int i : todo) {
        const int x = i / NY, y = i - x * NY;
        e.r0 = std::min(e.r0, x);
        e.r1 = std::max(e.r1, x);
        e.c0 = std::min(e.c0, y);
        e.c1 = std::max(e.c1, y);
    }
    const bool w = window();
    e.found = fits && w ? 1 : 0;
    if (visited) {
        std::sort(todo.begin(), todo.end());
        visited->swap(todo);
    }
    return e;
}

PlaneClear planClear(bool windowRun, const int win[4], const int prevRect[4], bool planesDirty, bool sweptDirty, bool splitPlanes) {
    if (planesDirty || sweptDirty) return PlaneClear::All;
    const bool same = win[1] > 0 && win[3] > 0 && std::equal(win, win + 4, prevRect);
    return (windowRun && same && !splitPlanes) ? PlaneClear::None : PlaneClear::Rect;
}


RunPlan planRun(const PathCaps& c, const PathRun& r) {
    RunPlan p;
    p.kind = r.kind;
    const bool run = r.kind == PathRun::Run;
    p.oneLaunch = c.stacked || ((c.merged == 1 || r.layerTiles) && c.mergedOk);
    p.plainMerged = plainMergedLaunch(c);
    p.layer = r.layerTiles;
    p.patch = c.usePatch && !r.layerTiles;
    const bool graph = !c.timeKernels && !c.streaming && (c.useGraph == 1 || (c.useGraph == 0 && c.ntiles <= 4096));
    const bool bandsWanted = run ? !graph : r.kind == PathRun::Raw;
    p.banded = bandsWanted && c.bands > 1 && !r.layerActive;
    p.segments = c.useSeg && !p.banded && !r.layerActive && r.segmentsFound;
    if (!run) return p;

    const bool smallWanted = c.smallGrid == 1 || (c.smallGrid == 0 && c.cells <= 1536);
    const bool small = smallWanted && !c.explicitTile && !c.timeKernels && c.useGraph != 1 && !c.streaming && c.smallFits &&
                       c.wholeWindow && !r.layerActive;
    p.reach = c.reachBound != 0 && p.plainMerged && !graph && !small && !c.useResident && !c.streaming && !p.banded && !p.segments &&
              !c.usePatch && !c.denseHistory && !c.edgeTiles && !c.slab && c.timeKernels == 0 && r.listenerInside;
    const bool resident = c.useResident && !(small && c.resident != 1) && !r.layerActive;
    const StepPath tiles = graph ? StepPath::Graph : StepPath::Launches;
    if (c.streaming) {
        p.path = StepPath::Streaming;
    } else if (p.reach && c.windowOk && !r.windowOff && !r.layerActive) {
        p.path = StepPath::Window;
    } else if (resident) {
        p.path = StepPath::Resident;
    } else if (small) {
        p.path = StepPath::SmallGrid;
    } else {
        p.path = tiles;
    }
    p.fallback = p.path == StepPath::Resident ? (small ? StepPath::SmallGrid : tiles)
                 : (p.path == StepPath::Window || p.path == StepPath::Graph) ? StepPath::Launches
                                                                             : p.path;
    return p;
}

}
```

### planeverb_amd/csrc/pv_core.h

```cpp
#pragma once

#include <cstdint>
#include <string>
#include <vector>

namespace pva {

constexpr float kC = 343.21f;
constexpr float kAudibleThreshold = 0.00000316f;
constexpr float kDryDirectionLen = 0.005f;
constexpr float kDryGainLen = 0.01f;
constexpr float kWetGainLen = 0.080f;
constexpr float kSqrt2 = 1.4142136f;
constexpr float kPointsPerWavelength = 3.5f;
constexpr float kSchroederOffset = 0.01f;
constexpr float kDistanceGainThreshold = 0.891251f;
constexpr float kDelayCloseThreshold = 5.f;
constexpr float kInvalidDryGain = -1.f;
constexpr int kLowResolution = 275;

struct GridSpec {
    int res = 0;
    float sizeX = 0, sizeY = 0;
    float dx = 0, dt = 0;
// ... 51 lines not shown
    float R = 0.f;
    float r = 0.f;
};
bool makeShape(const float* xy, int n, float R, Shape* out, std::string* err);
bool makeRound(const float* xy, int n, float radius, float R, Shape* out, std::string* err);
bool makePolygon(const float* xy, int n, float R, Shape* out, std::string* err);
bool polygonSelfIntersects(const float* xy, int n);
bool orientedBoxVertices(float px, float py, float w, float h, float ax, float ay, float out8[8], std::string* err);
bool shapeCovers(const Shape& s, float dx, int x, int y);
void shapeCellBounds(const Shape& s, const GridSpec& g, int* x0, int* x1, int* y0, int* y1);

constexpr int kMeshMax = 64;
constexpr int kMeshMaxTris = 1 << 20;
constexpr int kMeshMaxTrisTotal = 1 << 22;
enum MeshMode : int { kMeshSolid = 0, kMeshShell = 1 };
bool validateMesh(const float* verts, int nv, const int* tris, int nt, float R, int mode, float radius, std::string* err);
bool validateMeshTransform(const float* m12, std::string* err);
void meshSection(const float* verts, const int* tris, int nt, const float* m12, float h, float* out4, uint8_t* valid);
void meshCoverage(const GridSpec& g, const float* seg4, const uint8_t* valid, int nt, int mode, float radius, uint8_t* cover);
int meshCrossingPrefix(float xi, float dx, int gx);

constexpr int kEdgeLayerMaxWidth = 64;
constexpr int kEdgeLayerMinInterior = 8;
constexpr int kEdgeLayerDefaultWidth = 24;
constexpr double kEdgeLayerR0 = 0.1;
constexpr double kEdgeLayerSplitR0 = 1e-4;

void edgeLayerTables(int gx, int gy, float courant, const int w4[4], float* out, double r0 = kEdgeLayerR0);
inline bool edgeLayerR0Ok(double r0) { return r0 > 0.0 && r0 < 1.0; }
const char* edgeLayerRefusal(int gx, int gy, const int w4[4]);

bool loadPv(const std::string& path, std::vector<Box>* out, std::string* err);
bool savePv(const std::string& path, const std::vector<std::pair<int, Box>>& boxes, std::string* err);

void reverbBusGains(float rt60, float wet, float* a, float* b, float* c);

struct SegRect {
    int row0, nrows, tj0, w;
};
std::vector<SegRect> planSegments(const uint8_t* air, int ntx, int nty, int rxi, int wmax, int target);

struct Enclosure {
    int found;
    int cells;
    int r0, c0, r1, c1;
    int ti0, tj0, tis, tjs;
};
Enclosure findEnclosure(const uint8_t* beta, int NX, int NY, int seedX, int seedY, int rxi, int wi, int maxTiles,
                        std::vector<int>* visited);

enum class PlaneClear { None = 0, Rect = 1, All = 2 };
PlaneClear planClear(bool windowRun, const int win[4], const int prevRect[4], bool planesDirty, bool sweptDirty, bool splitPlanes);

struct PathCaps {
    bool stacked = false;
    bool mergedOk = false;
    bool smallFits = false;
    int useGraph = 0;
    int smallGrid = 0;
    int resident = 0;
    int merged = 1;
    int reachBound = -1;
    int timeKernels = 0;
    bool streaming = false, denseHistory = false, edgeTiles = false;
    bool explicitTile = false;
    bool slab = false;
    int ntiles = 0;
    long long cells = 0;
    int bands = 1;
    bool wholeWindow = false;
    bool useSeg = false, usePatch = false, windowOk = false;
    bool useResident = false;
};

struct PathRun {
    enum Kind { Run, Raw, Shared };
    Kind kind = Run;
    bool listenerInside = false;
    bool layerActive = false;
    bool layerTiles = false;
    bool windowOff = false;
    bool segmentsFound = true;
};

enum class StepPath { Streaming, Window, Resident, SmallGrid, Graph, Launches };

struct RunPlan {
    StepPath path = StepPath::Launches;
    StepPath fallback = StepPath::Launches;
    bool oneLaunch = false;
    bool plainMerged = false;
    bool banded = false;
    bool segments = false;
    bool patch = false;
    bool reach = false;
    bool layer = false;
    PathRun::Kind kind = PathRun::Run;
    bool oneXcd = false;
};

inline bool plainMergedLaunch(const PathCaps& c) { return !c.stacked && c.merged == 1 && c.mergedOk; }
RunPlan planRun(const PathCaps& c, const PathRun& r);

}
```

### planeverb_amd/csrc/pv_device.h

```cpp
#pragma once

#include <hip/hip_runtime.h>

#include <cstdint>

namespace pva {

constexpr float kCDev = 343.21f;
constexpr float kAudibleThresholdDev = 0.00000316f;
constexpr float kDistanceGainDev = 0.891251f;
constexpr float kDelayCloseDev = 5.f;

struct FaceCoef {
    float kx, ky, beta;
};
constexpr uint32_t kAirFaceBits = 0x7fc00000u;

struct Geometry {
    int gx, gy, NX, NY;
    int G;
    int rxi, wi;
    int ntx, nty;
    int rows, pitch;
    int x0, NXg, gxg;
};

struct DynParams {
    int lrow, lcol;
    int histRow0, histCol0;
    int histTileX0, histTileY0, histTilesX, histTilesY;
    int numGeneral;
    int numSeg;
};

struct SegDesc {
    int row0, nrows, tj0, w;
};

struct StepArgs {
    const float* prIn;
    const float* vxIn;
    const float* vyIn;
    float* prOut;
    float* vxOut;
    float* vyOut;
    const FaceCoef* coef;
    const float* pulse;
    float* hist;
    int* tileFirst;
    const uint8_t* tileClass;
    const uint8_t* tileDead;
    const int* generalList;
    int numGeneral;
    const SegDesc* segList;
    int numSeg;
    const DynParams* dyn;
    int* errFlag;
// ... 13 lines not shown
    int patchStrip;
    long long* patchTrace;
    int t0;
    int histSlot;
    int nsteps;
    int withPulse;
    int record;
    int dense;
    float courant;
    int inBytes;
    int sweepReverse;
    int reach;
    int reachGrow;
    int reachRow, reachCol;
    int winTi0, winTj0, winTis, winTjs;
};

__host__ __device__ inline bool tileInReach(int ti, int tj, int rxi, int wi, int G, int grow, int lrow, int lcol, int R) {
    const int r0 = G + ti * rxi - grow, r1 = G + (ti + 1) * rxi - 1 + grow;
    const int c0 = G + tj * wi - grow, c1 = G + (tj + 1) * wi - 1 + grow;
    const int dx = lrow < r0 ? r0 - lrow : (lrow > r1 ? lrow - r1 : 0);
    const int dy = lcol < c0 ? c0 - lcol : (lcol > c1 ? lcol - c1 : 0);
    return dx + dy <= R;
}

constexpr int kBatchMax = 8;
struct BatchArgs {
    int n;
    int gblocks;
    StepArgs a[kBatchMax];
};

struct BeginArgs {
    const DynParams* dynHost;
    DynParams* dyn;
    const int* listHost;
    int* list;
    const SegDesc* segHost;
    SegDesc* seg;
    int segCap;
    int* tileFirst;
    uint8_t* nz0;
    uint8_t* nz1;
    uint8_t* tileOpen;
    int* errFlag;
    int ntiles;
    int tileFirstInit;
    int listCap;
    const DynParams* dynBandsHost;
    DynParams* dynBands;
    int nbands;
    unsigned* zeroWords;
    int nZero;
};

struct SmallArgs {
    float* prOut;
    float* vxOut;
    float* vyOut;
    const FaceCoef* coef;
    const float* pulse;
    float* hist;
    const DynParams* dyn;
    long long histPlane;
    int histPitch;
    int pitch, G;
    int NX, NY;
    int T;
    int record;
    float courant;
    int rxi, wi;
};

struct ResidentArgs {
    float* pr[2];
    float* vx[2];
    float* vy[2];
    const FaceCoef* coef;
    const float* pulse;
    float* hist;
    int* tileFirst;
    DynParams dynVal;
    DynParams* dynOut;
    int* errFlag;
    unsigned* flags;
    int xcdMode;
    int xcdTarget;
    long long histPlane;
    long long planeBytes;
    int pitch, G;
    int ntx, nty, ntiles;
    int T;
    float courant;
    unsigned long long* stamp;
    int histSub;
    int winTi0, winTj0;
    int gridNty;
    int winRow0, winCol0;
    int window;
};

struct HaloHandoff {
    unsigned* count;
    unsigned* raise[2];
    const unsigned* await[2];
    unsigned seq;
// ... 6 lines not shown
    float* sEdry;
    float* sFx;
    float* sFy;
    uint8_t* cellsOpen2;
    const int* openList;
    const int* openCount;
    int* nextCount;
    int nDir, nDry;
    int gxRes, gyRes;
};

struct ClassifyArgs {
    const uint8_t* tileClass;
    const uint8_t* tileEmit;
    const uint8_t* tileOpenRing;
    const uint8_t* nzPrev;
    const uint8_t* cellsOpen2;
    const DynParams* dyn;
    uint8_t* classOut;
    uint8_t* ringOpenOut;
    uint8_t* nzNext;
    int* openList;
    int* openCount;
    int ntx, nty, G, K, rxi, wi, rows;
    int withPulse;
};

constexpr int kRt60WaveMaxCells = 12288;
constexpr int kRt60TileMinCells = 49152;

struct FarInfo {
    int on;
    int r0, c0, nr, nc;
    int gy;
    float lx, lz, dx;
    const int* box;
};

struct AnalyzeArgs {
    const unsigned* abortWord;
    const float* hist;
    const FaceCoef* coef;
    const int* tileFirst;
    const DynParams* dyn;
    float* out;
    float* delay;
    long long resN;
    long long histPlane;
    int histPitch;
    int pitch, G;
    int gx, gy;
    int rxi, wi, nty;
    int winRows, winCols;
    int* activeCount;
    int* unitList;
    int* dirScratch;
    int dirJump;
    int rt60Lanes;
    int rt60Tile;
    int T;
    int nDir, nDry, nWet, nCut;
    unsigned fs;
    int res;
    float dx;
    float courant;
    float efree;
    float lx, lz;
    int lcx, lcy;
    int x0;
    const float* histAbove;
    int lazyFar;
    int prevR0, prevC0, prevNR, prevNC;
    int* box;
    int* prevBox;
    unsigned long long* stamp;
    const int* labels;
    int labelNY;
    int wholeWindow;
    int ring;
    int tA, tB;
    int* sOnset;
    float* sEdry;
    float* sFx;
    float* sFy;
    float* sVx;
    float* sVy;
    uint8_t* tileOpenOut;
    const uint8_t* fuseClass;
    const uint8_t* fuseEmit;
    int fuseK;
    const int* ringList;
    int numRing;
    const int* emCells;
    float* emTrace;
    int numEmitters;
    float* recTrace;
    int recCols, recVel;
};

constexpr int kFusedCtlWords = 16;
struct FusedArgs {
    AnalyzeArgs a;
    unsigned* ctl;
    const float* carrySrc;
    int* errFlag;
};
// ... 3 lines not shown
```

### planeverb_amd/csrc/pv_rt60.hip

```cpp
#include <hip/hip_runtime.h>

#include <algorithm>
#include <cfloat>
#include <climits>
#include <cstdint>

#include "pv_analysis.h"
#include "pv_analysis_dev.h"
#include "pv_device.h"
#include "pv_launch.h"
#include "pv_libm.h"
#include "pv_prims.h"

#ifndef PV_RT60_TILE_NB
#define PV_RT60_TILE_NB 4
#endif
#ifndef PV_RT60_TILE_BLOCK
#define PV_RT60_TILE_BLOCK 256
#endif

namespace pva {

namespace {

// ... 156 lines not shown
#pragma unroll
        for (int k = 0; k < S; ++k) {
            edc = edc + p[k] * p[k];
            e[k] = edc;
        }
#pragma unroll
        for (int k = 0; k < S; ++k) {
            const int ii = i0 - k;
            const bool regress = live && ii >= sp && ii < endPoint;
            const float y = 10.f * pvLog10fNonNegT(regress ? e[k] : 1.f, ltab);
            xysum = regress ? xysum + y * (float)(ii - sp) : xysum;
            ysum = regress ? ysum + y : ysum;
        }
    }
    if (live) a.out[2 * a.resN + cell] = rt60FromSums(a, sp, xysum, ysum);
}

}

namespace {
__global__ __launch_bounds__(256) void pv_carry_results_kernel(const AnalyzeArgs a, const float* __restrict__ src, int r0, int c0,
                                                               int nr, int nc) {
    const int wc = blockIdx.x * blockDim.x + threadIdx.x, wr = blockIdx.y;
    int X, Y;
    if (nr < 0) {
        const DynParams dyn = *a.dyn;
        if (wc >= a.winCols) return;
        X = dyn.histRow0 - a.G + wr, Y = dyn.histCol0 - a.G + wc;
    } else {
        if (wc >= nc || wr >= nr) return;
        X = r0 + wr, Y = c0 + wc;
    }
    if (X < 0 || Y < 0 || X >= a.gx || Y >= a.gy) return;
    const long long s = (long long)X * a.gy + Y;
    if (a.delay[s] != FLT_MAX) return;
    a.out[s] = src[s];
    a.out[a.resN + s] = src[a.resN + s];
    a.out[2 * a.resN + s] = src[2 * a.resN + s];
    a.out[3 * a.resN + s] = src[3 * a.resN + s];
    a.out[6 * a.resN + s] = src[6 * a.resN + s];
    a.out[7 * a.resN + s] = src[7 * a.resN + s];
}
}

void launchCarryResults(const AnalyzeArgs& a, const float* srcOut, int srcR0, int srcC0, int srcNR, int srcNC, hipStream_t stream) {
    hipLaunchKernelGGL(pv_carry_results_kernel, dim3((a.winCols + 255) / 256, a.winRows), dim3(256), 0, stream, a, srcOut, 0, 0, -1,
                       0);
    if (srcNR > 0 && srcNC > 0)
        hipLaunchKernelGGL(pv_carry_results_kernel, dim3((unsigned)((srcNC + 255) / 256), (unsigned)srcNR), dim3(256), 0, stream, a,
                           srcOut, srcR0, srcC0, srcNR, srcNC);
}

void launchRt60Forms(const AnalyzeArgs& a, hipStream_t stream) {
    const long long groups = (a.histPlane + 63) / 64;
    hipLaunchKernelGGL(pv_rt60_groups_kernel, dim3((unsigned)std::min<long long>(4 * groups, a.rt60Lanes ? 8192 : 2048)), dim3(256), 0, stream, a);
    if (a.rt60Tile)
        hipLaunchKernelGGL((pv_rt60_tile_kernel<PV_RT60_TILE_S, PV_RT60_TILE_NB>),
                           dim3((unsigned)((a.histPlane + PV_RT60_TILE_BLOCK - 1) / PV_RT60_TILE_BLOCK)), dim3(PV_RT60_TILE_BLOCK), 0, stream, a);
}

}
```

### planeverb_amd/csrc/pv_run.hip

```cpp
#include <hip/hip_runtime.h>

#include "pv_device.h"
#include "pv_launch.h"
#include "pv_prims.h"
namespace pva {

__global__ void pv_begin_run_kernel(BeginArgs a) {
    const int i = blockIdx.x * blockDim.x + threadIdx.x;
    const int n = min(a.dynHost->numGeneral, a.listCap);
    if (i < n) a.list[i] = a.listHost[i];
    if (a.segHost && i < min(a.dynHost->numSeg, a.segCap)) a.seg[i] = a.segHost[i];
    if (i == 0) {
        *a.dyn = *a.dynHost;
        *a.errFlag = 0;
    }
    if (i < a.nbands) a.dynBands[i] = a.dynBandsHost[i];
    if (i < a.nZero) a.zeroWords[i] = 0u;
    if (a.tileFirst && i < a.ntiles) {
        a.tileFirst[i] = a.tileFirstInit;
        a.nz0[i] = 0;
        a.nz1[i] = 0;
        if (a.tileOpen) a.tileOpen[i] = 1;
    }
}

__global__ void pv_zero_kernel(float4* p, long long n4) {
    const long long i = (long long)blockIdx.x * blockDim.x + threadIdx.x;
    if (i < n4) p[i] = make_float4(0.f, 0.f, 0.f, 0.f);
}
void launchZero(float* p, long long n, hipStream_t stream) {
    const long long n4 = n / 4;
    hipLaunchKernelGGL(pv_zero_kernel, dim3((unsigned)((n4 + 255) / 256)), dim3(256), 0, stream, (float4*)p, n4);
}

__global__ void pv_zero_rect_kernel(ZeroRectArgs z) {
    const int i = blockIdx.x * blockDim.x + threadIdx.x;
    if (i >= z.nr * z.nc) return;
    const int r = i / z.nc;
    z.p[blockIdx.y][(long long)(z.r0 + r) * z.pitch + z.c0 + (i - r * z.nc)] = 0.f;
}
void launchZeroRect(const ZeroRectArgs& z, hipStream_t stream) {
    if (z.nr <= 0 || z.nc <= 0) return;
    hipLaunchKernelGGL(pv_zero_rect_kernel, dim3((unsigned)((z.nr * z.nc + 255) / 256), 6), dim3(256), 0, stream, z);
}

void launchBeginRun(const BeginArgs& a, hipStream_t stream) {
    int n = a.ntiles > a.listCap ? a.ntiles : a.listCap;
    if (a.segHost && a.segCap > n) n = a.segCap;
    if (a.nZero > n) n = a.nZero;
    hipLaunchKernelGGL(pv_begin_run_kernel, dim3((n + 255) / 256), dim3(256), 0, stream, a);
}


constexpr int kSmallThreads = 1024;
constexpr int kSmallCpt = 12;
constexpr int kSmallLdsBytes = 160 * 1024;

__host__ __device__ inline int smallLdsFloats(int NX, int NY) { return 3 * ((NX + 2) * NY + 2); }

bool smallGridFits(int NX, int NY) {
    return NX * NY <= kSmallThreads * kSmallCpt && smallLdsFloats(NX, NY) * 4 <= kSmallLdsBytes;
}

__global__ __launch_bounds__(kSmallThreads) void pv_small_grid_kernel(const SmallArgs a) {
    extern __shared__ __attribute__((aligned(16))) float smem[];
    const int NX = a.NX, NY = a.NY;
    const int cells = NX * NY;
    const int plane = (NX + 2) * NY + 2;
    float* sp = smem + NY;
// ... 89 lines not shown
```

### planeverb_amd/csrc/pv_solver.cpp

```cpp
#include "pv_solver.h"
#include "pv_boundary.h"
#include "pv_layer.h"
#include "pv_shapes.h"
#include "pv_mesh.h"

#include <unistd.h>

#include <algorithm>
#include <atomic>
#include <chrono>
#include <climits>
#include <cmath>
#include <cstdlib>
#include <cstring>
#include <limits>
#include <memory>
#include <mutex>

#include "pv_launch.h"
#include "pv_bands.h"
#include "pv_modulation.h"
#include "pv_decay.h"
#include "pv_echo.h"
#include "pv_echogram.h"
// ... 258 lines not shown
    geo_.wi = wi_;
    geo_.ntx = tileRow1 - tileRow0_;
    geo_.nty = ceilDiv(g_.NY, wi_);
    geo_.rows = kGuard + geo_.ntx * rxi_ + kGuard;
    geo_.pitch = roundUp(kGuard + geo_.nty * wi_ + kGuard, 64);
    const size_t plane = (size_t)geo_.rows * geo_.pitch;
    if (plane * 12 > (size_t)INT_MAX) return fail("grid too large for 32-bit plane offsets (12 bytes per cell of face coefficients)");
    const int ntiles = geo_.ntx * geo_.nty;

    {
        float* d = nullptr;
        if (!dalloc(&d, 128, true)) return false;
        launchLaneSelfTest(d, stream_);
        float h[128];
        if (!hipOk(hipMemcpyAsync(h, d, sizeof(h), hipMemcpyDeviceToHost, stream_), "selftest copy")) return false;
        if (!hipOk(hipStreamSynchronize(stream_), "selftest sync")) return false;
        hipFree(d);
        deviceBytes_ -= 128 * 4;
        for (int i = 0; i < 63; ++i)
            if (h[i] != (float)(i + 1)) return fail("DPP wave_shl self-test failed");
        for (int i = 1; i < 64; ++i)
            if (h[64 + i] != (float)(i - 1)) return fail("DPP wave_shr self-test failed");
    }

    for (int i = 0; i < 2; ++i) {
        if (!dalloc(&pr_[i], 3 * plane, true)) return false;
        vx_[i] = pr_[i] + plane;
        vy_[i] = pr_[i] + 2 * plane;
    }
    if (!dalloc(&coef_, plane, true)) return false;
    if (!dalloc(&matDev_, (size_t)g_.NX * g_.NY, true)) return false;
    if (!dalloc(&pulseDev_, (size_t)std::max(T_, g_.T), true)) return false;
    if (!dalloc(&tileFirst_, (size_t)ntiles, true)) return false;
    if (!dalloc(&tileClass_, (size_t)ntiles, true)) return false;
    if (!dalloc(&tileDead_, (size_t)ntiles, true) || !dalloc(&deadCount_, 1, true)) return false;
    if (!dalloc(&nz_[0], (size_t)ntiles, true) || !dalloc(&nz_[1], (size_t)ntiles, true)) return false;
    listCap_ = ntiles;
    if (!dalloc(&generalList_, (size_t)listCap_, true)) return false;
    if (!dalloc(&generalCount_, 1, true)) return false;
    if (!dalloc(&dynDev_, 1, true)) return false;
    if (!dalloc(&errFlag_, 1, true)) return false;
    if (!dalloc(&activeCount_, 8, true)) return false;
    if (!dalloc(&res_, (size_t)std::max(lgx_, 1) * g_.gy * 8, true)) return false;
    if (!dalloc(&delay_, (size_t)std::max(lgx_, 1) * g_.gy, true)) return false;
    lazyFar_ = opt_.lazyFar && !isSlab() && !opt_.streaming;
    if (lazyFar_) launchFillDelay(delay_, (long long)std::max(lgx_, 1) * g_.gy, stream_);
    {
        const char* e = getenv("PLANEVERB_AMD_NEAR_BOX");
        useNearBox_ = lazyFar_ && !(e && atoi(e) == 0);
        if (useNearBox_) {
            if (!dalloc(&nearBox_, 8, false)) return false;
            const int empty[8] = {INT_MAX, INT_MAX, -1, -1, INT_MAX, INT_MAX, -1, -1};
            if (!hipOk(hipMemcpyAsync(nearBox_, empty, sizeof(empty), hipMemcpyHostToDevice, stream_), "near box")) return false;
        }
    }
    scratchCount_ = std::max<size_t>({(size_t)3 * std::max(T_, g_.T), (size_t)lNX_ * g_.NY * 3,
                                     (size_t)geo_.ntx * rxi_ * geo_.nty * wi_});
    if (!dalloc(&scratch_, scratchCount_, true)) return false;

    {
        const int reach = T_ + 2 + K_;
        int wtx = geo_.ntx, wty = geo_.nty;
        histTilesXG_ = ntxG_;
        if (!opt_.denseHistory && !opt_.streaming) {
            histTilesXG_ = std::min(ntxG_, ceilDiv(2 * reach + 1, rxi_) + 1);
            wtx = std::min(geo_.ntx, histTilesXG_);
            wty = std::min(geo_.nty, ceilDiv(2 * reach + 1, wi_) + 1);
        }
        histTilesX_ = wtx;
        histTilesY_ = wty;
        histRows_ = wtx * rxi_;
        histPitch_ = roundUp(wty * wi_, 64);
        histPlane_ = (long long)wtx * wty * rxi_ * wi_;
        halfRing_ = std::min(roundUp(T_, K_), 8 * K_);
        ring_ = opt_.streaming ? 2 * halfRing_ : T_;
        const long long bytes = histPlane_ * 4 * (long long)ring_;
        if (histPlane_ * 4 > (long long)INT_MAX) return fail("history plane too large for 32-bit offsets");
        size_t freeB = 0, totalB = 0;
        hipMemGetInfo(&freeB, &totalB);
        if ((unsigned long long)bytes + (1ull << 30) > freeB)
            return fail("not enough HBM for the pressure history (" + std::to_string(bytes >> 20) +
                        " MiB for " + std::to_string(ring_) + " steps): use the sparse-emitter mode "
                        "(PVA_OPT_STREAMING_ANALYSIS + PvAmdSetEmitters), which keeps a 64-step ring instead");
        if (!hipOk(hipMalloc((void**)&hist_, (size_t)bytes), "hipMalloc history")) return false;
        deviceBytes_ += bytes;
        if (!dalloc(&unitList_, (size_t)(histPlane_ / 64 + 1), true)) return false;
        if (isSlab()) {
            if (opt_.slabIndex > 0 && !dalloc(&histAbove_, (size_t)T_ * histPitch_, true)) return false;
            if (opt_.slabIndex + 1 < opt_.slabCount && !dalloc(&histEdge_, (size_t)T_ * histPitch_, true)) return false;
        }
    }

    if (opt_.streaming) {
        const size_t nres = (size_t)g_.gx * g_.gy;
        if (!dalloc(&sOnset_, nres, true)) return false;
        for (auto& p : sState_)
            if (!dalloc(&p, nres, true)) return false;
        if (!dalloc(&tileOpen_, (size_t)ntiles, true) || !dalloc(&tileMarks_, (size_t)ntiles, true) ||
            !dalloc(&tileEmit_, (size_t)ntiles, true))
            return false;
        const bool fuseWanted = opt_.streamFuse > 0 || (opt_.streamFuse < 0 && ntiles >= 6000);
        streamFuse_ = fuseWanted && openConfigOk(K_, rxi_) && opt_.packed && opt_.merged == 1 && mergedConfigOk(K_, rxi_) &&
                      !stepConfigStacked(K_, rxi_) && opt_.timeKernels == 0;
        if (streamFuse_ && (!dalloc(&classStream_, (size_t)ntiles, true) || !dalloc(&ringOpen_, (size_t)ntiles, true) ||
                            !dalloc(&cellsOpen2_, (size_t)2 * ntiles, true) || !dalloc(&openList_, (size_t)2 * ntiles, true) ||
                            !dalloc(&openCount_, 2, true) || !dalloc(&ringList_, (size_t)ntiles, true) ||
// ... 960 lines not shown
                airChanged = airChanged || betaHost_[i] != (beta[i] ? 1 : 0);
                betaHost_[i] = beta[i] ? 1 : 0;
                byHost_[i] = mat_.by()[i];
            }
        if (!hipOk(hipMemcpyAsync((shapesActive_ ? matBaseDev_ : matDev_) + (size_t)lo * g_.NY, matHost_.data() + (size_t)lo * g_.NY,
                                  (size_t)(hi - lo) * g_.NY * sizeof(float), hipMemcpyHostToDevice, stream_),
                   "material upload"))
            return false;
    }
    if (meshActive_ && !composeMeshes(lo, hi)) return false;
    if (shapesActive_ && !composeShapes(lo, hi, &airChanged)) return false;
    launchCoefs(matDev_, coef_, geo_, stream_);
    if (!boundaryAbsorbing()) launchEdgeCoefs(coef_, geo_, edgeAdmittance(edgeR_), stream_);
    if (!hipOk(hipMemsetAsync(generalCount_, 0, sizeof(int), stream_), "memset")) return false;
    launchTileClass(K_, rxi_, coef_, tileClass_, generalList_, generalCount_, geo_, stream_,
                    opt_.edgeTiles);
    if (!hipOk(hipMemsetAsync(deadCount_, 0, sizeof(int), stream_), "memset")) return false;
    launchTileDead(coef_, tileDead_, deadCount_, geo_, K_, stream_);
    int count = 0;
    if (!hipOk(hipMemcpyAsync(&numDead_, deadCount_, sizeof(int), hipMemcpyDeviceToHost, stream_), "count copy"))
        return false;
    if (!hipOk(hipMemcpyAsync(&count, generalCount_, sizeof(int), hipMemcpyDeviceToHost, stream_), "count copy"))
        return false;
    if (!hipOk(hipStreamSynchronize(stream_), "geometry sync")) return false;
    if (shapesActive_) composeMirrors(&airChanged);
    wallTiles_.resize((size_t)count);
    if (count > 0 &&
        !hipOk(hipMemcpyAsync(wallTiles_.data(), generalList_, sizeof(int) * (size_t)count, hipMemcpyDeviceToHost, stream_),
               "list copy"))
        return false;
    tileClassHost_.resize((size_t)geo_.ntx * geo_.nty);
    if (!hipOk(hipMemcpyAsync(tileClassHost_.data(), tileClass_, tileClassHost_.size(), hipMemcpyDeviceToHost, stream_),
               "class copy") ||
        !hipOk(hipStreamSynchronize(stream_), "geometry sync"))
        return false;
    std::sort(wallTiles_.begin(), wallTiles_.end());
    if (!classifyLayer()) return false;
    count = (int)wallTiles_.size();
    {
        const char* e = getenv("PLANEVERB_AMD_GENERAL_PACKED");
        const long long nt = (long long)geo_.ntx * geo_.nty;
        stepWhich_ = 4 | (((e ? atoi(e) != 0 : (long long)count * 100 >= 8 * nt)) ? kStepGeneralPacked : 0);
    }
    if (airChanged) {
        enclosures_.clear();
        windowOff_ = false;
    }
    if ((airChanged || !labelsValid_) && !makeLabels()) return false;
    mat_.clearDirty();
    geometryDirty_ = false;
    boundaryDirty_ = false;
    layerDirty_ = false;
    planesDirty_ = true;
    dynValid_ = false;
    dropGraph();
    tim_.geometryMs =
        std::chrono::duration<float, std::milli>(std::chrono::steady_clock::now() - t0).count();
    return true;
}

bool Solver::makeLabels() {
    const size_t n = (size_t)g_.NX * g_.NY;
    if (isSlab() || opt_.streaming || opt_.skipAnalysis || n > (size_t)PV_LABEL_MAX_CELLS) return labelsValid_ = true;
    if (!labelDev_ && !dalloc(&labelDev_, n, false)) return false;
    labelHost_.assign(n, -1);
    std::vector<int> stack;
    int next = 0;
    const int NX = g_.NX, NY = g_.NY;
    for (size_t seed = 0; seed < n; ++seed) {
        if (!betaHost_[seed] || labelHost_[seed] >= 0) continue;
        labelHost_[seed] = next;
        stack.push_back((int)seed);
        while (!stack.empty()) {
            const int i = stack.back();
            stack.pop_back();
            const int x = i / NY, y = i - x * NY;
            const int nb[4] = {x > 0 ? i - NY : -1, x + 1 < NX ? i + NY : -1, y > 0 ? i - 1 : -1, y + 1 < NY ? i + 1 : -1};
            for (int j : nb)
                if (j >= 0 && betaHost_[(size_t)j] && labelHost_[(size_t)j] < 0) {
                    labelHost_[(size_t)j] = next;
                    stack.push_back(j);
                }
        }
        ++next;
    }
    labelsValid_ = hipOk(hipMemcpyAsync(labelDev_, labelHost_.data(), n * sizeof(int), hipMemcpyHostToDevice, stream_), "label upload") &&
                   hipOk(hipStreamSynchronize(stream_), "label sync");
    return labelsValid_;
}


bool Solver::freeFieldEnergyAt(int cellX, int cellY, int n, float r, float* out) {
    const int hr = cellX + geo_.G - dynCur_.histRow0, hc = cellY + geo_.G - dynCur_.histCol0;
    const int hti = hr / rxi_, htj = hc / wi_;
    const long long off = ((long long)(hti * histTilesY_ + htj) * rxi_ + (hr - hti * rxi_)) * wi_ + (hc - htj * wi_);
    launchEfree(hist_, histPlane_, off, n, r, scratch_, stream_);
    if (!hipOk(hipMemcpyAsync(out, scratch_, 4, hipMemcpyDeviceToHost, stream_), "efree copy")) return false;
    return hipOk(hipStreamSynchronize(stream_), "efree sync");
}

bool Solver::computeEfree() {
    const int lx0 = g_.gx / 2, ly0 = g_.gy / 2;
    const int ex = lx0 + (int)(1.f / g_.dx), ey = ly0;
    int lcx, lcy;
    listenerCell(g_, (float)lx0 * g_.dx, (float)ly0 * g_.dx, &lcx, &lcy);
    const int n = g_.nFree;
// ... 89 lines not shown
        int pos = 0, b = 0;
        bandListOff_[0] = 0;
        for (int t : all) {
            const int ti = t / geo_.nty;
            while (ti >= bandRow_[(size_t)b + 1]) {
                ++b;
                bandListOff_[(size_t)b] = pos;
            }
            listHost_[pos++] = (ti - bandRow_[(size_t)b]) * geo_.nty + (t - ti * geo_.nty);
        }
        while (b < nb_) bandListOff_[(size_t)++b] = pos;
        for (int k = 0; k < nb_; ++k) {
            bandListCount_[(size_t)k] = bandListOff_[(size_t)k + 1] - bandListOff_[(size_t)k];
            DynParams v = d;
            const int r0 = bandRow_[(size_t)k];
            if (inside) v.lrow -= r0 * rxi_;
            v.histTileX0 -= r0;
            v.histRow0 -= r0 * rxi_;
            v.numGeneral = bandListCount_[(size_t)k];
            dynBandsHost_[k] = v;
        }
    }
    dynValid_ = true;
    return true;
}

void Solver::buildSegments(int listed) {
    const int ntx = geo_.ntx, nty = geo_.nty;
    std::vector<uint8_t> air((size_t)ntx * nty);
    for (size_t t = 0; t < air.size(); ++t) air[t] = tileClassHost_[t] == 0;
    for (int i = 0; i < listed; ++i) air[(size_t)listHost_[i]] = 0;
    const std::vector<SegRect> segs = planSegments(air.data(), ntx, nty, rxi_, segWMax_, opt_.segments > 0 ? opt_.segments : 1024);
    int n = 0;
    for (const SegRect& r : segs) {
        if (n >= segCap_) break;
        segHost_[n++] = SegDesc{r.row0, r.nrows, r.tj0, r.w};
    }
    numSeg_ = n;
}

bool Solver::zeroPlanesIfNeeded() {
    if (numDead_ == 0 || !planesDirty_) return true;
    const size_t bytes = (size_t)geo_.rows * geo_.pitch * 4;
    for (int i = 0; i < 2; ++i)
        if (!hipOk(hipMemsetAsync(pr_[i], 0, bytes, stream_), "plane clear") ||
            !hipOk(hipMemsetAsync(vx_[i], 0, bytes, stream_), "plane clear") ||
            !hipOk(hipMemsetAsync(vy_[i], 0, bytes, stream_), "plane clear") ||
            (px_[i] && !hipOk(hipMemsetAsync(px_[i], 0, bytes, stream_), "plane clear")))
            return false;
    planesDirty_ = false;
    return true;
}

void Solver::enqueueBeginRun(bool resetTiles) {
    BeginArgs b{};
    b.dynHost = dynHost_;
    b.dyn = dynDev_;
    b.listHost = listHost_;
    b.list = generalList_;
    b.tileFirst = resetTiles ? tileFirst_ : nullptr;
    b.nz0 = nz_[0];
    b.nz1 = nz_[1];
    b.tileOpen = opt_.streaming ? tileOpen_ : nullptr;
    b.errFlag = errFlag_;
    b.ntiles = geo_.ntx * geo_.nty;
    b.tileFirstInit = opt_.denseHistory ? 0 : INT_MAX;
    b.listCap = listCap_;
    b.segHost = plan_.segments ? segHost_ : nullptr;
    b.seg = segList_;
    b.segCap = segCap_;
    b.dynBandsHost = plan_.banded ? dynBandsHost_ : nullptr;
    b.dynBands = dynBandsDev_;
    b.nbands = plan_.banded ? nb_ : 0;
    b.zeroWords = resFlags_;
    b.nZero = resFlags_ ? resFlagWords_ : 0;
    launchBeginRun(b, stream_);
}

StepArgs Solver::baseStepArgs(bool withPulse, bool record) const {
    StepArgs a{};
    a.coef = coef_;
    a.pulse = pulseDev_;
    a.hist = hist_;
    a.tileFirst = tileFirst_;
    a.tileClass = tileClass_;
    a.tileDead = (record && numDead_ > 0) ? tileDead_ : nullptr;
    a.generalList = generalList_;
    a.numGeneral = launchCap_;
    a.segList = plan_.segments ? segList_ : nullptr;
    a.numSeg = plan_.segments ? numSeg_ : 0;
    a.dyn = dynDev_;
    a.tileOpen = opt_.streaming ? tileOpen_ : nullptr;
    a.errFlag = errFlag_;
    a.histPlane = histPlane_;
    a.planeBytes = (long long)geo_.rows * geo_.pitch * 4;
    a.histPitch = histPitch_;
    a.pitch = geo_.pitch;
    a.G = geo_.G;
    a.ntx = geo_.ntx;
    a.nty = geo_.nty;
    a.ntiles = geo_.ntx * geo_.nty;
    a.gx = g_.gx;
    a.gy = g_.gy;
    a.bandRows = ceilDiv(geo_.ntx, 8);
    a.tileOrder = opt_.tileOrder;
    a.patchStrip = opt_.patchStrip;
    a.patchTrace = patchTrace_;
    a.packed = opt_.packed ? 1 : 0;
// ... 49 lines not shown
    reachRect_[3] = a.winTjs;
}

const Enclosure* Solver::enclosureOf(int lcx, int lcy) {
    if (lcx < 0 || lcx >= g_.NX || lcy < 0 || lcy >= g_.NY || !betaHost_[(size_t)lcx * g_.NY + lcy]) return nullptr;
    const int cell = lcx * g_.NY + lcy;
    for (const EnclosureRec& r : enclosures_)
        if (lcx >= r.e.r0 && lcx <= r.e.r1 && lcy >= r.e.c0 && lcy <= r.e.c1 && std::binary_search(r.cells.begin(), r.cells.end(), cell))
            return &r.e;
    if (enclosures_.size() >= 16) enclosures_.erase(enclosures_.begin());
    enclosures_.emplace_back();
    EnclosureRec& r = enclosures_.back();
    r.e = findEnclosure(betaHost_.data(), g_.NX, g_.NY, lcx, lcy, rxi_, wi_, std::min(residentBudget_, kResidentMaxTiles) / 3, &r.cells);
    return &r.e;
}

static bool reserveBlocks(std::atomic<int>& inFlight, int blocks, int budget, int* held) {
    if (inFlight.fetch_add(blocks) + blocks > budget) {
        inFlight.fetch_sub(blocks);
        return false;
    }
    *held = blocks;
    return true;
}

bool Solver::windowFor(int lcx, int lcy, int win[4]) {
    if (probeWindow_) {
        if (!reserveBlocks(residentInFlight(device_), 3, residentBudget_, &residentHeld_)) return false;
        win[0] = win[2] = 0;
        win[1] = win[3] = 1;
        return true;
    }
    const Enclosure* e = enclosureOf(lcx, lcy);
    if (!e || !e->found) return false;
    const DynParams& d = dynCur_;
    if (e->ti0 < d.histTileX0 || e->ti0 + e->tis > d.histTileX0 + d.histTilesX || e->tj0 < d.histTileY0 ||
        e->tj0 + e->tjs > d.histTileY0 + d.histTilesY || e->ti0 + e->tis > geo_.ntx || e->tj0 + e->tjs > geo_.nty)
        return false;
    const int blocks = 3 * e->tis * e->tjs;
    if (blocks > std::min(residentBudget_, kResidentMaxTiles)) return false;
    if (!reserveBlocks(residentInFlight(device_), blocks, residentBudget_, &residentHeld_)) return false;
    win[0] = e->ti0;
    win[1] = e->tis;
    win[2] = e->tj0;
    win[3] = e->tjs;
    return true;
}

void Solver::enqueueWindowRun(const int win[4]) {
    const int blocks = 3 * win[1] * win[3];
    plan_.oneXcd = xcdOk_ && (xcdWindowOk_ || probeWindow_) && blocks <= kResidentXcdMaxTiles &&
                   reserveBlocks(residentXcdInFlight(device_, xcdTarget_), blocks, kResidentXcdMaxTiles, &xcdHeld_);
    runTiles_ = blocks;
    enqueueBeginRun(true);
    launchResidentRun(12, win);
    for (int i = 0; i < 4; ++i) reachRect_[i] = win[i];
}

void Solver::launchResidentRun(int tileRows, const int* win) {
    if (stampTimed()) stampsHost_[0] = stampsHost_[1] = stampsHost_[2] = 0ull;
    launchResident(K_, tileRows, residentArgs(win), stream_);
    tim_.stepLaunches = ceilDiv(T_, K_);
    cur_ = tim_.stepLaunches & 1;
}

ResidentArgs Solver::residentArgs(const int* win) const {
    const long long off = win ? (long long)win[0] * rxi_ * geo_.pitch + (long long)win[2] * wi_ : 0;
    ResidentArgs ra{};
    for (int i = 0; i < 2; ++i) {
        ra.pr[i] = pr_[i] + off;
        ra.vx[i] = vx_[i] + off;
        ra.vy[i] = vy_[i] + off;
    }
    ra.coef = coef_ + off;
    ra.pulse = pulseDev_;
    ra.hist = hist_;
    ra.tileFirst = tileFirst_;
    ra.dynVal = dynCur_;
    ra.dynOut = dynDev_;
    ra.errFlag = errFlag_;
    ra.flags = resFlags_;
    ra.xcdMode = plan_.oneXcd ? 1 : 0;
    ra.xcdTarget = xcdTarget_;
    ra.histPlane = histPlane_;
    ra.planeBytes = ((long long)geo_.rows * geo_.pitch - off) * 4;
    ra.pitch = geo_.pitch;
    ra.G = geo_.G;
    ra.ntx = win ? 3 * win[1] : geo_.ntx;
    ra.nty = win ? win[3] : geo_.nty;
    ra.ntiles = ra.ntx * ra.nty;
    ra.T = T_;
    ra.courant = g_.courant;
    ra.stamp = stampTimed() ? stampsHost_ : nullptr;
    ra.histSub = win ? 3 : 1;
    ra.gridNty = geo_.nty;
    if (win) {
        ra.winTi0 = win[0];
        ra.winTj0 = win[2];
        ra.winRow0 = win[0] * rxi_;
        ra.winCol0 = win[2] * wi_;
        ra.window = 1;
    }
    return ra;
}

bool Solver::clearReachPlanes(const int* win) {
    float* planes[6] = {pr_[0], vx_[0], vy_[0], pr_[1], vx_[1], vy_[1]};
// ... 291 lines not shown
    a.sOnset = sOnset_;
    a.sEdry = sState_[0];
    a.sFx = sState_[1];
    a.sFy = sState_[2];
    a.sVx = sState_[3];
    a.sVy = sState_[4];
    a.fuseClass = streamFuse_ ? tileClass_ : nullptr;
    a.fuseEmit = tileEmit_;
    a.fuseK = K_;
    a.ringList = streamFuse_ ? ringList_ : nullptr;
    a.numRing = numRing_;
    a.emCells = emCells_;
    a.emTrace = emTrace_;
    a.numEmitters = numEmitters_;
    a.recTrace = recTrace_;
    a.recCols = recCols_;
    a.recVel = recVel_ ? 1 : 0;
    a.tileOpenOut = tileMarks_;
    return a;
}

Solver::Block Solver::curWindow() const {
    Block b;
    b.r0 = dynCur_.histRow0 - geo_.G;
    b.c0 = dynCur_.histCol0 - geo_.G;
    b.nr = std::max(0, std::min(histTilesX_ * rxi_, g_.gx - b.r0));
    b.nc = std::max(0, std::min(histTilesY_ * wi_, g_.gy - b.c0));
    return b;
}

FarInfo Solver::farInfo() const {
    FarInfo f{};
    f.on = (lazyFar_ && dynValid_ && !farDirValid_) ? 1 : 0;
    f.r0 = farWin_.r0;
    f.c0 = farWin_.c0;
    f.nr = farWin_.nr;
    f.nc = farWin_.nc;
    f.box = (f.on && nearBoxValid_) ? nearBox_ + 4 * nearPar_ : nullptr;
    f.gy = g_.gy;
    f.lx = lastLx_;
    f.lz = lastLz_;
    f.dx = g_.dx;
    return f;
}

bool Solver::ensureFarDirections() {
    if (!lazyFar_ || farDirValid_ || !dynValid_) return true;
    launchFarDirections(res_, (long long)g_.gx * g_.gy, farInfo(), stream_);
    farDirValid_ = true;
    return hipOk(hipGetLastError(), "far directions");
}

void Solver::enqueueAnalysis(float lx, float lz) {
    const AnalyzeArgs a = analyzeArgs(lx, lz);
    const bool carry = carryFrom_ && carryFrom_ != this && carryFrom_->device_ == device_ && !opt_.streaming && !isSlab();
    if (carry) hipStreamWaitEvent(stream_, carryFrom_->ev_[2], 0);
    if (useFused_) {
        FusedArgs f{};
        f.a = a;
        f.ctl = fusedCtl_;
        f.carrySrc = carry ? carryFrom_->res_ : nullptr;
        f.errFlag = errFlag_;
        launchAnalysisFused(f, stream_);
        if (lazyFar_) {
            farWin_ = curWindow();
            farDirValid_ = false;
        }
        nearBoxValid_ = false;
        return;
    }
    launchAnalysisFar(a, stream_);
    launchOnset(a, stream_);
    const bool fork = opt_.analysisFork == 2 || (opt_.analysisFork != 0 && histPlane_ >= kAnalysisForkCells);
    if (fork) {
        hipEventRecord(anaEv_[0], stream_);
        hipStreamWaitEvent(stream2_, anaEv_[0], 0);
        launchRt60(a, stream2_);
        hipEventRecord(anaEv_[1], stream2_);
        launchEncode(a, stream_);
    } else {
        launchEncode(a, stream_);
        launchRt60(a, stream_);
    }
    if (carry) {
        Block w = carryFrom_->dynValid_ ? carryFrom_->curWindow() : Block{};
        const Block mine = curWindow();
        if (w.r0 == mine.r0 && w.c0 == mine.c0 && w.nr == mine.nr && w.nc == mine.nc) w = Block{};
        launchCarryResults(a, carryFrom_->res_, w.r0, w.c0, w.nr, w.nc, stream_);
    }
    launchAnalysisDirection(a, stream_);
    if (fork) hipStreamWaitEvent(stream_, anaEv_[1], 0);
    if (lazyFar_) {
        farWin_ = curWindow();
        farDirValid_ = false;
    }
    if (a.box) nearPar_ ^= 1;
    nearBoxValid_ = a.box != nullptr;
}

bool Solver::beginRun(PathRun::Kind kind, int lcx, int lcy, bool withPulse, float lx, float lz) {
    if (pendingTimings_ && !sync()) return false;
    invalidateAnalysisMaps();
    lastRun_ = LastRun::Failed;
    for (RecordSet& r : recs_) r.run = RecordSet::Run::None;
    if (!applyGeometry()) return false;
    PathRun r;
    r.kind = kind;
    r.listenerInside = withPulse && lcx >= 0 && lcx <= g_.gx && lcy >= 0 && lcy <= g_.gy;
    r.layerActive = layerActive();
    r.layerTiles = numLayer_ > 0;
    r.windowOff = windowOff_;
    plan_ = planRun(caps_, r);
    if (!prepareDyn(lcx, lcy, withPulse)) return false;
    if (plan_.segments && numSeg_ == 0) {
        r.segmentsFound = false;
        plan_ = planRun(caps_, r);
    }
    tim_.stepLaunches = 0;
    kevUsed_ = 0;
    launchCap_ = numGeneral_;
    if (kind == PathRun::Raw) {
        planesDirty_ = true;
        return true;
    }
    if (!zeroPlanesIfNeeded()) return false;
    lastLx_ = lx;
    lastLz_ = lz;
    cur_ = 0;
    if (plan_.reach) return true;
    sweptDirty_ = true;
    return true;
}

bool Solver::enqueueRun(int lcx, int lcy, float lx, float lz) {
    const auto inUse = queue_.lockUse();
    if (!hipOk(hipSetDevice(device_), "hipSetDevice")) return false;
    if (!beginRun(PathRun::Run, lcx, lcy, true, lx, lz)) return false;
    if (plan_.path == StepPath::Streaming) return enqueueStreamingRun(lx, lz);
    lastLcx_ = lcx;
    lastLcy_ = lcy;
    releaseResident();
    int win[4] = {0, 0, 0, 0};
    if (plan_.path == StepPath::Window && !windowFor(lcx, lcy, win)) plan_.path = plan_.fallback;
    if (plan_.path == StepPath::Resident && !reserveBlocks(residentInFlight(device_), caps_.ntiles, residentBudget_, &residentHeld_))
        plan_.path = plan_.fallback;
    if (plan_.reach && !clearReachPlanes(plan_.path == StepPath::Window && !repeating_ ? win : nullptr)) return false;
    if (!stampTimed()) hipEventRecord(ev_[0], stream_);
    switch (plan_.path) {
        case StepPath::Window: enqueueWindowRun(win); break;
        case StepPath::Resident: enqueueResidentRun(); break;
        case StepPath::SmallGrid:
            if (!enqueueSmallGridRun()) return false;
            break;
        case StepPath::Graph:
            if (!enqueueGraphRun()) return false;
            break;
        case StepPath::Launches:
            if (!enqueueResetAndSteps()) return false;
            break;
        case StepPath::Streaming: break;
    }
    if (!stampTimed()) hipEventRecord(ev_[1], stream_);
    if (!opt_.skipAnalysis) enqueueAnalysis(lx, lz);
    if (!stampTimed()) hipEventRecord(ev_[2], stream_);
    lastRunBatched_ = false;
    enqueueQueryRecords();
    enqueueQuerySpectralRecords();
    launchRunFinish(res_, (long long)g_.gx * g_.gy, qCellsHost_, opt_.skipAnalysis ? 0 : numQueries_, qOutHost_, farInfo(), errFlag_,
                    activeCount_, plan_.oneXcd ? resFlags_ + runTiles_ + 1 : nullptr, statusHost_, resFlags_,
                    resFlags_ ? resFlagWords_ : 0, stampTimed() ? stampsHost_ : nullptr, stream_);
    if (stampTimed()) hipEventRecord(ev_[2], stream_);
    enqueueTap();
    statusQueued_ = true;
    pendingTimings_ = true;
    return hipOk(hipGetLastError(), "run launch");
}

bool Solver::enqueueStreamingRun(float lx, float lz) {
    const int ntiles = geo_.ntx * geo_.nty;
    hipEventRecord(ev_[0], stream_);
    const size_t nres = (size_t)g_.gx * g_.gy;
    if (!hipOk(hipMemsetAsync(sOnset_, 0xff, nres * 4, stream_), "state reset")) return false;
    for (float* p : sState_)
        if (!hipOk(hipMemsetAsync(p, 0, nres * 4, stream_), "state reset")) return false;
    if (numEmitters_ > 0 &&
        !hipOk(hipMemsetAsync(emTrace_, 0, (size_t)numEmitters_ * T_ * 4, stream_), "trace reset"))
        return false;
    if (streamFuse_ && (!hipOk(hipMemsetAsync(cellsOpen2_, 1, (size_t)2 * ntiles, stream_), "open flags") ||
                        !hipOk(hipMemsetAsync(openCount_, 0, 2 * sizeof(int), stream_), "open count")))
        return false;
    enqueueBeginRun(true);
    if (streamFuse_) {
        std::vector<uint8_t> in((size_t)ntiles, 0);
        int n = 0;
        auto add = [&](int t) {
            if (!in[(size_t)t]) {
                in[(size_t)t] = 1;
                ringHost_[n++] = t;
            }
        };
        for (int i = 0; i < numGeneral_; ++i) add(listHost_[i]);
        for (int t = 0; t < ntiles; ++t)
// ... 582 lines not shown
}

bool Solver::uploadTileEmit() {
    const int ntiles = geo_.ntx * geo_.nty;
    emTilesHost_.assign((size_t)ntiles, 0);
    zoneTileUnion(emitterTilesHost_.empty() ? nullptr : emitterTilesHost_.data(), zoneTilesHost_.empty() ? nullptr : zoneTilesHost_.data(),
                  ntiles, emTilesHost_.data());
    return hipOk(hipMemcpyAsync(tileEmit_, emTilesHost_.data(), emTilesHost_.size(), hipMemcpyHostToDevice, stream_), "emitter tiles");
}

bool Solver::impulseResponse(int cx, int cy, float* out3T) {
    if (opt_.streaming) return fail("the full pressure history is not kept in streaming-analysis mode");
    if (cx < 0 || cx >= lNX_ || cy < 0 || cy > g_.gy) return fail("cell outside the grid");
    if (!dynValid_) return fail("no simulation has run yet");
    if (!hipOk(hipSetDevice(device_), "hipSetDevice")) return false;
    launchIr(analyzeArgs(lastLx_, lastLz_), cx, cy, scratch_, stream_);
    if (!hipOk(hipMemcpyAsync(out3T, scratch_, (size_t)3 * T_ * 4, hipMemcpyDeviceToHost, stream_), "ir copy"))
        return false;
    return hipOk(hipStreamSynchronize(stream_), "ir sync");
}

bool Solver::impulseResponseCells(int cx, int cy, void* out16T) {
    std::vector<float> f((size_t)3 * T_);
    if (!impulseResponse(cx, cy, f.data())) return false;
    struct RefCell {
        float pr, vx, vy;
        short b, by;
    };
    static_assert(sizeof(RefCell) == 16, "PvTypes.h:106-121");
    const size_t i = (size_t)(cx + x0_) * g_.NY + cy;
    const short b = (short)betaHost_[i], by = (short)byHost_[i];
    RefCell* out = static_cast<RefCell*>(out16T);
    for (int t = 0; t < T_; ++t) out[t] = RefCell{f[(size_t)3 * t], f[(size_t)3 * t + 1], f[(size_t)3 * t + 2], b, by};
    return true;
}

bool Solver::copyFields(float* pr, float* vx, float* vy) {
    if (!hipOk(hipSetDevice(device_), "hipSetDevice")) return false;
    const size_t n = (size_t)lNX_ * g_.NY;
    const float* src[3] = {pr_[cur_], vx_[cur_], vy_[cur_]};
    float* dst[3] = {pr, vx, vy};
    for (int i = 0; i < 3; ++i) {
        if (!dst[i]) continue;
        launchUnpad(src[i], scratch_, geo_, stream_);
        if (!hipOk(hipMemcpyAsync(dst[i], scratch_, n * 4, hipMemcpyDeviceToHost, stream_), "field copy")) return false;
        if (!hipOk(hipStreamSynchronize(stream_), "field sync")) return false;
    }
    return true;
}

bool Solver::setFields(const float* pr, const float* vx, const float* vy) {
    if (isSlab()) return fail("setFields is not available on a slab");
    planesDirty_ = true;
    if (!hipOk(hipSetDevice(device_), "hipSetDevice")) return false;
    const size_t n = (size_t)g_.NX * g_.NY;
    const float* src[3] = {pr, vx, vy};
    float* dst[3] = {pr_[cur_], vx_[cur_], vy_[cur_]};
    const size_t planeBytes = (size_t)geo_.rows * geo_.pitch * 4;
    for (float* p : px_)
        if (p && !hipOk(hipMemsetAsync(p, 0, planeBytes, stream_), "field clear")) return false;
    for (int i = 0; i < 3; ++i) {
        if (!hipOk(hipMemsetAsync(dst[i], 0, planeBytes, stream_), "field clear")) return false;
        if (!src[i]) continue;
        if (!hipOk(hipMemcpyAsync(scratch_, src[i], n * 4, hipMemcpyHostToDevice, stream_), "field upload")) return false;
        launchPad(scratch_, dst[i], geo_, stream_);
        if (!hipOk(hipStreamSynchronize(stream_), "field sync")) return false;
    }
    return true;
}

bool Solver::copyHistoryPlane(int t, float* pr) {
    if (opt_.streaming) return fail("the full pressure history is not kept in streaming-analysis mode");
    if (t < 0 || t >= T_) return fail("step outside the recorded range");
    if (!dynValid_) return fail("no simulation has run yet");
    if (!hipOk(hipSetDevice(device_), "hipSetDevice")) return false;
    launchHistPlane(analyzeArgs(lastLx_, lastLz_), t, scratch_, lNX_, g_.NY, histRows_, stream_);
    if (!hipOk(hipMemcpyAsync(pr, scratch_, (size_t)lNX_ * g_.NY * 4, hipMemcpyDeviceToHost, stream_), "plane copy"))
        return false;
    return hipOk(hipStreamSynchronize(stream_), "plane sync");
}

bool Solver::setHistoryPlane(int t, const float* pr) {
    if (isSlab()) return fail("set history plane: not available on a slab");
    if (opt_.streaming) return fail("set history plane: the full pressure history is not kept in streaming-analysis mode");
    if (t < 0 || t >= T_) return fail("set history plane: step outside the recorded range");
    const auto inUse = queue_.lockUse();
    if (!hipOk(hipSetDevice(device_), "hipSetDevice")) return false;
    if (pendingTimings_ && !sync()) return false;
    if (lastRun_ == LastRun::None || !dynValid_) return fail("set history plane: no completed run");
    if (lastRun_ != LastRun::Ok) return fail("set history plane: the last run ended in error");
    invalidateAnalysisMaps();
    if (!hipOk(hipMemcpyAsync(scratch_, pr, (size_t)g_.NX * g_.NY * 4, hipMemcpyHostToDevice, stream_), "set history plane upload"))
        return false;
    launchSetHistPlane(analyzeArgs(lastLx_, lastLz_), t, scratch_, g_.NX, g_.NY, histRows_, hist_, stream_);
    return hipOk(hipGetLastError(), "set history plane launch") && hipOk(hipStreamSynchronize(stream_), "set history plane sync");
}

bool Solver::copyPulse(float* out) {
    std::memcpy(out, pulse_.data(), (size_t)g_.T * 4);
    return true;
}

bool Solver::copyMaterial(uint8_t* beta, float* R) {
    const size_t n = (size_t)g_.NX * g_.NY;
    if (shapesActive_) {
        if (!hipOk(hipSetDevice(device_), "hipSetDevice") || !applyGeometry()) return false;
// ... 11 lines not shown
```

### planeverb_amd/csrc/pv_solver.h

```cpp
#pragma once

#include <hip/hip_runtime.h>

#include <cstdint>
#include <memory>
#include <mutex>
#include <string>
#include <vector>

#include "pv_core.h"
#include "pv_device.h"
#include "pv_query_spectral.h"
#include "pv_zone_decay.h"
#include "pv_zone_maps.h"

namespace pva {

struct SolverOptions {
    int K = 0;
    int rxi = 0;
    bool denseHistory = false;
    int numSteps = 0;
    bool skipAnalysis = false;
    int useGraph = 0;
    bool withFreeGrid = true;
    int tileOrder = -1;
    int merged = 1;
    int segments = 0;
    bool streaming = false;
    bool autoStreaming = false;
    bool packed = true;
    bool edgeTiles = false;
    int smallGrid = 0;
    int timeKernels = 0;
    int slabIndex = 0, slabCount = 1;
    int auxStreams = 0;
    int streamFuse = -1;
    bool lazyFar = true;
    int patch = -1;
    int patchStrip = 3;
    int streamPriority = 0;
    bool debugLoseFirstCapture = false;
    int fusedAnalysis = -1;
    int analysisFork = 1;
    int rt60Lanes = 0;
    int resident = 0;
    int xcdRegions = -1;
    int alternateSweeps = -1;
    int rowBands = 0;
    int reachBound = -1;
    int residentWindow = -1;
};

struct SolverTimings {
    float fdtdMs = 0, analysisMs = 0, geometryMs = 0;
    float stepLoopMs = 0;
    float airKernelMs = 0, generalKernelMs = 0;
    int airLaunches = 0, generalLaunches = 0;
    int stepLaunches = 0;
    int reachedCells = 0;
    int activeCells = 0;
    int silentCells = 0;
};

enum AnalysisKind {
    kMapRoomMetrics,
    kMapDecayTimes,
    kMapLateralFraction,
    kMapEchoCriterion,
    kMapEchogram,
    kMapLobes,
    kMapBandMetrics,
    kMapModulation,
    kMapSpectrum,
    kAnalysisKinds
};

class SlabGroup;
class SlabRoot;
struct SlabRankOps;

struct QueueClaim {
    std::vector<hipStream_t> parked;
    hipStream_t claimed = nullptr;
    int redeals = 0;
    std::shared_ptr<std::recursive_mutex> use;
    std::unique_lock<std::recursive_mutex> lockUse() const { return use ? std::unique_lock<std::recursive_mutex>(*use) : std::unique_lock<std::recursive_mutex>(); }
    enum { kNormal = 0, kHigh = 1, kLow = 2 };
    bool claim(int device, hipStream_t* stream, int priority, const void* owner);
    bool replace(hipStream_t* stream);
    int priorityClass = kNormal;
    void release();
};

struct RunTap {
    virtual ~RunTap() = default;
    virtual void afterRun(const float* res, const float* delay, long long resN, int gy, int r0, int c0, int nr, int nc,
                          hipStream_t stream) = 0;
};

class Solver {
    friend class SlabGroup;
    friend class SlabRoot;
    friend struct SlabRankOps;

public:
    static Solver* create(const GridSpec& spec, int device, const SolverOptions& opt, std::string* err);
    ~Solver();

    const GridSpec& spec() const { return g_; }
    const Geometry& geometry() const { return geo_; }
    int device() const { return device_; }
    int K() const { return K_; }
    int rxi() const { return rxi_; }
    float efree() const { return efree_; }
    void setEfree(float e) { efree_ = e; }
    int T() const { return T_; }
    long long deviceBytes() const { return deviceBytes_; }
    int histRows() const { return histRows_; }
    int histPitch() const { return histPitch_; }
    const std::string& lastError() const { return err_; }
    bool streamFuse() const { return streamFuse_; }
    bool lastRunResidentWindow() const { return plan_.path == StepPath::Window; }
    bool lastRunOneXcd() const { return plan_.oneXcd; }
    bool residentKernel() const { return caps_.useResident && !layerActive(); }
    SolverOptions& options() { return opt_; }

    int addBox(const Box& b);
    bool updateBox(int id, const Box& b);
    bool removeBox(int id);
    int numBoxes() const;
    std::vector<std::pair<int, Box>> boxes() const;
    void rasterAdd(const Box& b) {
        mat_.add(b);
        invalidateAnalysisMaps();
    }
    void rasterRemove(const Box& b) {
        mat_.remove(b);
        invalidateAnalysisMaps();
    }

    int addShape(const Shape& sh);
    bool updateShape(int id, const Shape& sh);
    bool removeShape(int id);
    int numShapes() const;
    bool shapeSet(int id, const Shape& sh);
    bool shapeClear(int id);

    int addMesh(const float* verts, int nv, const int* tris, int nt, float R, int mode, float radius);
    bool updateMesh(int id, const float* verts, int nv, const int* tris, int nt, float R, int mode, float radius);
    bool setMeshTransform(int id, const float* m12);
    bool removeMesh(int id);
    int numMeshes() const;
    int meshTriangles(int id) const;
    bool setSliceHeight(float h);
    float sliceHeight() const { return sliceH_; }
    bool copyMeshSection(int id, float* out4, uint8_t* valid);
    bool meshSet(int id, const float* verts, int nv, const int* tris, int nt, float R, int mode, float radius);
    bool meshClear(int id);

    bool setGridBoundary(const float R4[4]);
    void gridBoundary(float R4[4]) const;
    bool boundaryAbsorbing() const;

    bool setEdgeLayer(const int w4[4], bool split = false, double r0 = kEdgeLayerR0);
    void edgeLayer(int w4[4]) const;
    void edgeLayerModel(bool* split, double* r0) const {
        *split = layerSplit_;
        *r0 = layerR0_;
    }
    bool layerActive() const { return layerW_[0] > 0 || layerW_[1] > 0 || layerW_[2] > 0 || layerW_[3] > 0; }

    bool run(float lx, float ly, float lz, bool wait, Solver* carryFrom = nullptr);
    bool runCells(int lcx, int lcy, float lx, float lz, bool wait);
    bool sync();
    static bool runBatch(Solver* const* s, int n, const float* lxyz, bool wait, std::string* err);
// ... 74 lines not shown
    int arrays(int* count, int cap, int* interp) const;
    int arrayTapsOf(int array, int* memberIndex, int* delaySteps, float* weight, int cap);
    bool setArrayRecords(unsigned timeKinds, unsigned spectralKinds);
    void arrayRecordKinds(unsigned* timeKinds, unsigned* spectralKinds) const;
    int arrayRecordFloats(int family, unsigned kind);
    bool computeArrays(float* ms);
    bool copyArrayResponse(int array, float* outT);
    bool arrayOnsets(float* out, int nArrays);
    bool arrayRecords(int family, unsigned kind, float* out, int nArrays);
    bool setAuralisation(int rate, int zeroCrossings, float beta);
    bool auralisation(int* rate, int* zeroCrossings, float* beta, int* L, int* K) const;
    int auralTapsOf(int* first, float* w, int capN);
    bool computeAuralResponses(int source, const float* xyz, int nPos, float* ms);
    bool copyAuralResponse(int r, float* outL);
    bool setAuralForm(int form);
    bool auralise(const float* signals, int nSignals, int N, const int* route, const float* gain, float* ms);
    bool copyAuralOutput(int r, float* outM);
    bool copyAuralMix(float* outM);
    bool setZones(const unsigned char* labels, int nZones);
    int zones(unsigned char* labels) const;
    int zoneStatPlanes(AnalysisKind k) const;
    bool computeZoneStats(AnalysisKind k, void* out, int cap, float* ms, int* count);
    bool computeZoneDecay(int align, void* out, int cap, double* etc, double* edc, float* ms, int* count);
    int zoneDecayChunkSlots() const;
    bool setZoneCurves(bool on);
    bool zoneCurves() const;
    bool setZoneMaps(unsigned kinds);
    unsigned zoneMaps() const;
    bool computeZoneBandDecay(int align, void* out, int cap, double* etc, double* edc, float* ms, int* count);
    int zoneBandDecayChunks(int* slots, int* bands) const;
    bool copyPulse(float* out);
    bool copyMaterial(uint8_t* beta, float* R);
    bool freeFieldEnergyAt(int cellX, int cellY, int n, float r, float* out);
    bool setEmitters(const float* xyz, int n);

private:
    Solver() = default;
    bool init(const GridSpec& spec, int device, const SolverOptions& opt);
    bool applyGeometry();
    bool computeEfree();
    PathCaps caps_;
    RunPlan plan_;
    bool beginRun(PathRun::Kind kind, int lcx, int lcy, bool withPulse, float lx, float lz);
    bool enqueueRun(int lcx, int lcy, float lx, float lz);
    bool enqueueStreamingRun(float lx, float lz);
    void enqueueResidentRun();
    void launchResidentRun(int tileRows, const int* win);
    bool enqueueSmallGridRun();
    bool enqueueGraphRun();
    bool enqueueSteps(int firstStep, int nsteps, bool withPulse, bool record, bool fromZero = false);
    StepArgs baseStepArgs(bool withPulse, bool record) const;
    void setLaunchArgs(StepArgs& a, int t0, int k, bool firstOfRun, int li) const;
    bool prepareDyn(int lcx, int lcy, bool withPulse);
    void enqueueBeginRun(bool resetTiles);
    bool zeroPlanesIfNeeded();
    AnalyzeArgs analyzeArgs(float lx, float lz) const;
    bool lazyFar_ = false;
    struct Block {
        int r0 = 0, c0 = 0, nr = 0, nc = 0;
    };
    Block curWindow() const;
    Block farWin_;
    bool farDirValid_ = true;
    int* nearBox_ = nullptr;
    int nearPar_ = 0;
    bool useNearBox_ = false;
    bool nearBoxValid_ = false;
    unsigned long long* stampsHost_ = nullptr;
    bool stampTimed() const { return (plan_.path == StepPath::Resident || plan_.path == StepPath::Window) && stampsHost_; }
    bool labelsValid_ = false;
    int lastReached_ = -1;
    FarInfo farInfo() const;
    bool ensureFarDirections();
    void enqueueAnalysis(float lx, float lz);
    Solver* carryFrom_ = nullptr;
    RunTap* tap_ = nullptr;
    void enqueueTap();
    bool fail(const std::string& what);
    bool hipOk(hipError_t e, const char* what);
    template <typename Tp>
    bool dalloc(Tp** p, size_t count, bool zero);

    GridSpec g_;
    int x0_ = 0;
    int tileRow0_ = 0;
    int lNX_ = 0;
    int lgx_ = 0;
    int ntxG_ = 0, histTilesXG_ = 0;
    bool isSlab() const { return opt_.slabCount > 1; }
    int globalWindowTileRow0(int lcx) const;
    float* histAbove_ = nullptr;
    float* histEdge_ = nullptr;
    Geometry geo_{};
    SolverOptions opt_;
    int device_ = 0;
    int K_ = 4, rxi_ = 32, wi_ = 56;
    int T_ = 0;
    hipStream_t stream_ = nullptr;
    hipStream_t stream2_ = nullptr;
    bool lastRunBatched_ = false;
    std::vector<hipStream_t> auxStreams_;
    std::vector<hipEvent_t> airDone_, genDone_;
    int stepWhich_ = 4;
    QueueClaim queue_;
    bool redealMainStream() { return queue_.replace(&stream_); }
    hipEvent_t forkEv_ = nullptr;
    hipEvent_t anaEv_[2] = {nullptr, nullptr};
    hipGraph_t graph_ = nullptr;
    hipGraphExec_t graphExec_ = nullptr;
    int graphCap_ = -1;
    bool captureLossInjected_ = false;
    bool buildGraph(int cap);
    void dropGraph();
    bool enqueueResetAndSteps();
    hipEvent_t ev_[4] = {nullptr, nullptr, nullptr, nullptr};
    hipEvent_t pubEv_[2] = {nullptr, nullptr};
    bool pubCopyPending_ = false;
    long long deviceBytes_ = 0;
    std::string err_;

// ... 414 lines not shown
```

Baseline: 42720 billion.

## Restrict analysis kernels to resident-window cover instead of full history plane

Measured after the change: 44200 billion (median of 6 runs). 1.03x the previous value.

```diff
diff --git a/include/planeverb_amd.h b/include/planeverb_amd.h
--- a/include/planeverb_amd.h
+++ b/include/planeverb_amd.h
@@ -154,6 +154,7 @@
     PVA_OPT_XCD_REGIONS = 27,
     PVA_OPT_REACH_BOUND = 30,
     PVA_OPT_RESIDENT_WINDOW = 31,
+    PVA_OPT_ANALYSIS_COVER = 32,
     PVA_OPT_DEBUG_LOSE_FIRST_CAPTURE = 24,
     PVA_OPT_PATCH_STRIP = 18,
     PVA_OPT_EDGE_TILES = 15
@@ -262,6 +263,8 @@
                                   int* out10);
 PVA_EXPORT int PvAmdHostWindowClear(int windowRun, const int* win4, const int* prevRect4, int planesDirty, int sweptDirty,
                                     int splitPlanes);
+PVA_EXPORT int PvAmdHostAnalysisCover(const int* win4, const int* hist4, int tileRows, int tileCols, int prevKind,
+                                      const int* prevRect4, int* out, int outCap);
 PVA_EXPORT int PvAmdHostOrientedBoxVertices(float px, float py, float w, float h, float ax, float ay, float* out8);
 PVA_EXPORT int PvAmdHostShape(const float* xy, int n, float absorption, float* out16);
 PVA_EXPORT int PvAmdHostShapeCoverage(float gridSizeX, float gridSizeY, int gridResolution, const float* xy, int n,
@@ -294,6 +297,7 @@
 PVA_EXPORT int PvAmdLibmProbe(int form, const float* in, float* out, long long n, int onDevice);
 PVA_EXPORT int PvAmdGetTimings(PvAmdSolver* s, PvAmdTimings* out);
 PVA_EXPORT int PvAmdLastRunResidentWindow(PvAmdSolver* s);
+PVA_EXPORT int PvAmdLastRunAnalysisCover(PvAmdSolver* s);
 PVA_EXPORT int PvAmdLastRunOneXcd(PvAmdSolver* s);
 
 PVA_EXPORT int PvAmdSetEmitters(PvAmdSolver* s, const float* xyz, int n);
diff --git a/planeverb_amd/api.py b/planeverb_amd/api.py
--- a/planeverb_amd/api.py
+++ b/planeverb_amd/api.py
@@ -40,6 +40,7 @@
 PVA_OPT_FUSED_ANALYSIS = 29
 PVA_OPT_REACH_BOUND = 30
 PVA_OPT_RESIDENT_WINDOW = 31
+PVA_OPT_ANALYSIS_COVER = 32
 
 
 class PlaneverbOutput(C.Structure):
@@ -262,6 +263,9 @@
     "PvAmdGetTimings": (C.c_int, [_vp, C.POINTER(PvAmdTimings)]),
     "PvAmdLastRunResidentWindow": (C.c_int, [_vp]),
     "PvAmdLastRunOneXcd": (C.c_int, [_vp]),
+    "PvAmdLastRunAnalysisCover": (C.c_int, [_vp]),
+    "PvAmdHostAnalysisCover": (C.c_int, [C.POINTER(C.c_int), C.POINTER(C.c_int), C.c_int, C.c_int, C.c_int, C.POINTER(C.c_int),
+                                         C.POINTER(C.c_int), C.c_int]),
     "PvAmdHostWindowClear": (C.c_int, [C.c_int, C.POINTER(C.c_int), C.POINTER(C.c_int), C.c_int, C.c_int, C.c_int]),
     "PvAmdClockProbe": (C.c_float, [C.c_int, _fp]),
     "PvAmdBandwidthProbe": (C.c_int, [C.c_int, _fp]),
@@ -869,6 +873,22 @@
     return rc
 
 
+def host_analysis_cover(win, hist, tile_rows, tile_cols, prev=None):
+    w, h = ((C.c_int * 4)(*[int(v) for v in r]) for r in (win, hist))
+    kind = 0 if prev is None else 1 if isinstance(prev, str) else 2
+    if isinstance(prev, str) and prev != "empty":
+        raise ValueError("prev must be None, 'empty' or a cell rectangle")
+    p = (C.c_int * 4)(*([int(v) for v in prev] if kind == 2 else [0, 0, 0, 0]))
+    out = (C.c_int * 26)()
+    rc = lib().PvAmdHostAnalysisCover(w, h, int(tile_rows), int(tile_cols), kind, p, out, 26)
+    if rc < 0:
+        raise PlaneverbError(last_error())
+    if rc == 0:
+        return None
+    v = [int(x) for x in out]
+    return dict(runs=[(v[10 + 2 * r], v[11 + 2 * r]) for r in range(v[0])], groups=v[1], rect=tuple(v[2:6]), dir_rect=tuple(v[6:10]))
+
+
 def load_pv(path, max_boxes=4096):
     buf = np.empty((max_boxes, 5), np.float32)
     n = lib().PvAmdHostLoadPv(path.encode(), _f(buf), max_boxes)
@@ -1657,7 +1677,8 @@
                 "debug_lose_first_capture": PVA_OPT_DEBUG_LOSE_FIRST_CAPTURE, "stream_priority": PVA_OPT_STREAM_PRIORITY,
                 "alternate_sweeps": PVA_OPT_ALTERNATE_SWEEPS, "xcd_regions": PVA_OPT_XCD_REGIONS,
                 "analysis_fork": PVA_OPT_ANALYSIS_FORK, "fused_analysis": PVA_OPT_FUSED_ANALYSIS,
-                "reach_bound": PVA_OPT_REACH_BOUND, "resident_window": PVA_OPT_RESIDENT_WINDOW}
+                "reach_bound": PVA_OPT_REACH_BOUND, "resident_window": PVA_OPT_RESIDENT_WINDOW,
+                "analysis_cover": PVA_OPT_ANALYSIS_COVER}
         for k, v in options.items():
             _check(lib().PvAmdSetOption(self._h, keys[k], int(v)))
         self.info = PvAmdInfo()
@@ -1849,6 +1870,12 @@
         if rc < 0:
             raise PlaneverbError(last_error())
         return rc == 1
+
+    def last_run_analysis_cover(self):
+        rc = lib().PvAmdLastRunAnalysisCover(self._h)
+        if rc < 0:
+            raise PlaneverbError(last_error())
+        return rc
 
     def last_run_one_xcd(self):
         rc = lib().PvAmdLastRunOneXcd(self._h)
diff --git a/planeverb_amd/csrc/pv_analysis.h b/planeverb_amd/csrc/pv_analysis.h
--- a/planeverb_amd/csrc/pv_analysis.h
+++ b/planeverb_amd/csrc/pv_analysis.h
@@ -10,6 +10,9 @@
 namespace pva {
 
 __device__ __forceinline__ bool analysisAborted(const AnalyzeArgs& a) { return a.abortWord && *a.abortWord != 0u; }
+
+inline long long analysisGroups(const AnalyzeArgs& a) { return a.cover.runs ? a.cover.groups : (a.histPlane + 63) / 64; }
+inline long long analysisCells(const AnalyzeArgs& a) { return a.cover.runs ? (long long)a.cover.rows * a.cover.cols : a.histPlane; }
 
 struct NearBox {
     int r0, c0, r1, c1;
diff --git a/planeverb_amd/csrc/pv_analysis.hip b/planeverb_amd/csrc/pv_analysis.hip
--- a/planeverb_amd/csrc/pv_analysis.hip
+++ b/planeverb_amd/csrc/pv_analysis.hip
@@ -38,10 +38,33 @@
 
 __device__ __forceinline__ bool analysisWindowCell(const AnalyzeArgs& a, const DynParams& dyn, int* X, int* Y) {
     const int wc = blockIdx.x * blockDim.x + threadIdx.x, wr = blockIdx.y;
+    if (a.cover.runs) {
+        if (wc >= a.cover.dirCols) return false;
+        *X = a.cover.dirR0 + wr;
+        *Y = a.cover.dirC0 + wc;
+        return *X < a.gx && *Y < a.gy;
+    }
     if (wc >= a.winCols) return false;
     *X = dyn.histRow0 - a.G + wr;
     *Y = dyn.histCol0 - a.G + wc;
     return *X < a.gx && *Y < a.gy;
+}
+
+__device__ __forceinline__ int onsetGroup(const AnalysisCover& cv, const int b) {
+    int g = b, rem = b;
+    bool done = cv.runs == 0;
+#pragma unroll
+    for (int r = 0; r < kCoverMaxRuns; ++r) {
+        if (!done && r < cv.runs) {
+            if (rem < cv.runCount[r]) {
+                g = cv.runFirst[r] + rem;
+                done = true;
+            } else {
+                rem -= cv.runCount[r];
+            }
+        }
+    }
+    return g;
 }
 
 #ifndef PV_ONSET_WAVES
@@ -56,7 +79,8 @@
     if (analysisAborted(a)) return;
     const DynParams dyn = *a.dyn;
     const int lane = threadIdx.x & 63, wave = __builtin_amdgcn_readfirstlane((int)(threadIdx.x >> 6));
-    const long long g = (long long)blockIdx.x * 64 + lane;
+    const int group = onsetGroup(a.cover, (int)blockIdx.x);
+    const long long g = (long long)group * 64 + lane;
     const PlaneCell c = planeCell(a, dyn, g);
     const int T = a.T;
     int tF = INT_MAX;
@@ -163,7 +187,7 @@
     if (lane == 0) {
         if (mr) {
             atomicAdd(a.activeCount + 1, __popcll(mr));
-            a.unitList[atomicAdd(a.activeCount + 4, 1)] = (int)blockIdx.x;
+            a.unitList[atomicAdd(a.activeCount + 4, 1)] = group;
         }
         if (ms) atomicAdd(a.activeCount + 3, __popcll(ms));
     }
@@ -329,7 +353,10 @@
     forDirectionCells(a, dyn, [&](const int p) { dirFinalCell<false>(a, dyn, J, p); });
 }
 
-static dim3 analysisWindowGrid(const AnalyzeArgs& a) { return dim3((a.winCols + 255) / 256, a.winRows); }
+static dim3 analysisWindowGrid(const AnalyzeArgs& a) {
+    if (a.cover.runs) return dim3((a.cover.dirCols + 255) / 256, a.cover.dirRows);
+    return dim3((a.winCols + 255) / 256, a.winRows);
+}
 
 static void launchDirectionJump(const AnalyzeArgs& a, int* J, hipStream_t stream) {
     const dim3 grid = analysisWindowGrid(a), block(256);
@@ -349,16 +376,17 @@
 }
 
 void launchOnset(const AnalyzeArgs& a, hipStream_t stream) {
-    hipLaunchKernelGGL(pv_onset_kernel, dim3((unsigned)((a.histPlane + 63) / 64)), dim3(64 * kOnsetWaves), 0, stream, a);
+    hipLaunchKernelGGL(pv_onset_kernel, dim3((unsigned)analysisGroups(a)), dim3(64 * kOnsetWaves), 0, stream, a);
 }
 void launchEncode(const AnalyzeArgs& a, hipStream_t stream) {
-    const unsigned units = (unsigned)((a.histPlane + 63) / 64);
-    if (a.rt60Lanes != 1 && a.histPlane <= 16384)
+    const unsigned units = (unsigned)analysisGroups(a);
+    const long long cells = analysisCells(a);
+    if (a.rt60Lanes != 1 && cells <= 16384)
         hipLaunchKernelGGL(pv_encode_groups_kernel<16>, dim3(units * 4), dim3(256), 0, stream, a);
-    else if (a.rt60Lanes != 1 && a.histPlane <= kRt60TileMinCells)
+    else if (a.rt60Lanes != 1 && cells <= kRt60TileMinCells)
         hipLaunchKernelGGL(pv_encode_groups_kernel<4>, dim3(units), dim3(256), 0, stream, a);
     else
-        hipLaunchKernelGGL(pv_encode_kernel, dim3((unsigned)((a.histPlane + 255) / 256)), dim3(256), 0, stream, a);
+        hipLaunchKernelGGL(pv_encode_kernel, dim3((units + 3) / 4), dim3(256), 0, stream, a);
 }
 void launchRt60(const AnalyzeArgs& a, hipStream_t stream) { launchRt60Forms(a, stream); }
 
diff --git a/planeverb_amd/csrc/pv_capi.cpp b/planeverb_amd/csrc/pv_capi.cpp
--- a/planeverb_amd/csrc/pv_capi.cpp
+++ b/planeverb_amd/csrc/pv_capi.cpp
@@ -716,6 +716,7 @@
         case PVA_OPT_XCD_REGIONS: h->opt.xcdRegions = (int)value; break;
         case PVA_OPT_REACH_BOUND: h->opt.reachBound = (int)value; break;
         case PVA_OPT_RESIDENT_WINDOW: h->opt.residentWindow = (int)value; break;
+        case PVA_OPT_ANALYSIS_COVER: h->opt.analysisCover = (int)value; break;
         default: g_lastError = "unknown option"; return -1;
     }
     return 0;
@@ -1128,6 +1129,11 @@
 int PvAmdLastRunResidentWindow(PvAmdSolver* h) try {
     if (!wholeGrid(h) || !ensure(h, true)) return -1;
     return h->s->lastRunResidentWindow() ? 1 : 0;
+} PV_API_CATCH(-1)
+
+int PvAmdLastRunAnalysisCover(PvAmdSolver* h) try {
+    if (!wholeGrid(h) || !ensure(h, true)) return -1;
+    return h->s->lastRunAnalysisCover();
 } PV_API_CATCH(-1)
 
 int PvAmdLastRunOneXcd(PvAmdSolver* h) try {
@@ -2233,6 +2239,23 @@
     return (int)planClear(windowRun != 0, win4, prevRect4, planesDirty != 0, sweptDirty != 0, splitPlanes != 0);
 } PV_API_CATCH(-1)
 
+int PvAmdHostAnalysisCover(const int* win4, const int* hist4, int tileRows, int tileCols, int prevKind, const int* prevRect4,
+                           int* out, int outCap) try {
+    if (!win4 || !hist4 || !out || outCap < 10 + 2 * kCoverMaxRuns || (prevKind == 2 && !prevRect4)) {
+        g_lastError = "PvAmdHostAnalysisCover: bad arguments";
+        return -1;
+    }
+    AnalysisCover c{};
+    if (!planAnalysisCover(win4, hist4, tileRows, tileCols, prevKind, prevRect4, &c)) return 0;
+    const int head[10] = {c.runs, c.groups, c.r0, c.c0, c.rows, c.cols, c.dirR0, c.dirC0, c.dirRows, c.dirCols};
+    std::copy(head, head + 10, out);
+    for (int r = 0; r < kCoverMaxRuns; ++r) {
+        out[10 + 2 * r] = c.runFirst[r];
+        out[11 + 2 * r] = c.runCount[r];
+    }
+    return c.runs;
+} PV_API_CATCH(-1)
+
 int PvAmdHostLoadPv(const char* path, float* b5, int maxBoxes) try {
     if (!path) return -1;
     std::vector<Box> boxes;
diff --git a/planeverb_amd/csrc/pv_core.cpp b/planeverb_amd/csrc/pv_core.cpp
--- a/planeverb_amd/csrc/pv_core.cpp
+++ b/planeverb_amd/csrc/pv_core.cpp
@@ -763,6 +763,53 @@
     return (windowRun && same && !splitPlanes) ? PlaneClear::None : PlaneClear::Rect;
 }
 
+bool planAnalysisCover(const int win[4], const int hist[4], int rxi, int wi, int prevKind, const int prevRect[4], AnalysisCover* out) {
+    *out = AnalysisCover{};
+    const int ti0 = win[0], tis = win[1], tj0 = win[2], tjs = win[3];
+    const int hx0 = hist[0], hy0 = hist[1], hnx = hist[2], hny = hist[3];
+    if (rxi < 1 || wi < 1 || tis < 1 || tjs < 1 || hnx < 1 || hny < 1) return false;
+    if (tis > kCoverMaxRuns) return false;
+    if (ti0 < hx0 || ti0 + tis > hx0 + hnx || tj0 < hy0 || tj0 + tjs > hy0 + hny) return false;
+    const long long tileCells = (long long)rxi * wi;
+    if ((long long)hnx * hny * tileCells > std::numeric_limits<int>::max()) return false;
+    AnalysisCover c{};
+    c.r0 = ti0 * rxi;
+    c.c0 = tj0 * wi;
+    c.rows = tis * rxi;
+    c.cols = tjs * wi;
+    if (prevKind == 2) {
+        if (!prevRect) return false;
+        const bool empty = prevRect[2] <= 0 || prevRect[3] <= 0;
+        if (!empty && (prevRect[0] < c.r0 || prevRect[1] < c.c0 || prevRect[0] + prevRect[2] > c.r0 + c.rows ||
+                       prevRect[1] + prevRect[3] > c.c0 + c.cols))
+            return false;
+    } else if (prevKind != 1) {
+        return false;
+    }
+    long long last = -1;
+    for (int i = 0; i < tis; ++i) {
+        const long long cell0 = ((long long)(ti0 - hx0 + i) * hny + (tj0 - hy0)) * tileCells;
+        const long long g0 = cell0 / 64, g1 = (cell0 + tjs * tileCells - 1) / 64;
+        if (c.runs > 0 && g0 <= last + 1) {
+            c.runCount[c.runs - 1] += (int)(g1 - last);
+        } else {
+            if (c.runs == kCoverMaxRuns) return false;
+            c.runFirst[c.runs] = (int)g0;
+            c.runCount[c.runs] = (int)(g1 - g0 + 1);
+            ++c.runs;
+        }
+        last = g1;
+    }
+    for (int r = 0; r < c.runs; ++r) c.groups += c.runCount[r];
+    const int hr0 = hx0 * rxi, hc0 = hy0 * wi, hr1 = hr0 + hnx * rxi, hc1 = hc0 + hny * wi;
+    c.dirR0 = std::max(c.r0 - 1, hr0);
+    c.dirC0 = std::max(c.c0 - 1, hc0);
+    c.dirRows = std::min(c.r0 + c.rows + 1, hr1) - c.dirR0;
+    c.dirCols = std::min(c.c0 + c.cols + 1, hc1) - c.dirC0;
+    *out = c;
+    return true;
+}
+
 
 RunPlan planRun(const PathCaps& c, const PathRun& r) {
     RunPlan p;
diff --git a/planeverb_amd/csrc/pv_core.h b/planeverb_amd/csrc/pv_core.h
--- a/planeverb_amd/csrc/pv_core.h
+++ b/planeverb_amd/csrc/pv_core.h
@@ -127,6 +127,17 @@
 enum class PlaneClear { None = 0, Rect = 1, All = 2 };
 PlaneClear planClear(bool windowRun, const int win[4], const int prevRect[4], bool planesDirty, bool sweptDirty, bool splitPlanes);
 
+constexpr int kCoverMaxRuns = 8;
+struct AnalysisCover {
+    int runs;
+    int groups;
+    int runFirst[kCoverMaxRuns];
+    int runCount[kCoverMaxRuns];
+    int r0, c0, rows, cols;
+    int dirR0, dirC0, dirRows, dirCols;
+};
+bool planAnalysisCover(const int win[4], const int hist[4], int rxi, int wi, int prevKind, const int prevRect[4], AnalysisCover* out);
+
 struct PathCaps {
     bool stacked = false;
     bool mergedOk = false;
diff --git a/planeverb_amd/csrc/pv_device.h b/planeverb_amd/csrc/pv_device.h
--- a/planeverb_amd/csrc/pv_device.h
+++ b/planeverb_amd/csrc/pv_device.h
@@ -3,6 +3,8 @@
 #include <hip/hip_runtime.h>
 
 #include <cstdint>
+
+#include "pv_core.h"
 
 namespace pva {
 
@@ -122,6 +124,8 @@
     int nbands;
     unsigned* zeroWords;
     int nZero;
+    int byValue;
+    DynParams dynVal;
 };
 
 struct SmallArgs {
@@ -234,6 +238,7 @@
     int gx, gy;
     int rxi, wi, nty;
     int winRows, winCols;
+    AnalysisCover cover;
     int* activeCount;
     int* unitList;
     int* dirScratch;
diff --git a/planeverb_amd/csrc/pv_rt60.hip b/planeverb_amd/csrc/pv_rt60.hip
--- a/planeverb_amd/csrc/pv_rt60.hip
+++ b/planeverb_amd/csrc/pv_rt60.hip
@@ -232,11 +232,11 @@
 }
 
 void launchRt60Forms(const AnalyzeArgs& a, hipStream_t stream) {
-    const long long groups = (a.histPlane + 63) / 64;
+    const long long groups = analysisGroups(a);
     hipLaunchKernelGGL(pv_rt60_groups_kernel, dim3((unsigned)std::min<long long>(4 * groups, a.rt60Lanes ? 8192 : 2048)), dim3(256), 0, stream, a);
     if (a.rt60Tile)
         hipLaunchKernelGGL((pv_rt60_tile_kernel<PV_RT60_TILE_S, PV_RT60_TILE_NB>),
-                           dim3((unsigned)((a.histPlane + PV_RT60_TILE_BLOCK - 1) / PV_RT60_TILE_BLOCK)), dim3(PV_RT60_TILE_BLOCK), 0, stream, a);
-}
-
-}
+                           dim3((unsigned)((groups * 64 + PV_RT60_TILE_BLOCK - 1) / PV_RT60_TILE_BLOCK)), dim3(PV_RT60_TILE_BLOCK), 0, stream, a);
+}
+
+}
diff --git a/planeverb_amd/csrc/pv_run.hip b/planeverb_amd/csrc/pv_run.hip
--- a/planeverb_amd/csrc/pv_run.hip
+++ b/planeverb_amd/csrc/pv_run.hip
@@ -7,14 +7,21 @@
 
 __global__ void pv_begin_run_kernel(BeginArgs a) {
     const int i = blockIdx.x * blockDim.x + threadIdx.x;
-    const int n = min(a.dynHost->numGeneral, a.listCap);
-    if (i < n) a.list[i] = a.listHost[i];
-    if (a.segHost && i < min(a.dynHost->numSeg, a.segCap)) a.seg[i] = a.segHost[i];
-    if (i == 0) {
-        *a.dyn = *a.dynHost;
-        *a.errFlag = 0;
+    if (a.byValue) {
+        if (i == 0) {
+            *a.dyn = a.dynVal;
+            *a.errFlag = 0;
+        }
+    } else {
+        const int n = min(a.dynHost->numGeneral, a.listCap);
+        if (i < n) a.list[i] = a.listHost[i];
+        if (a.segHost && i < min(a.dynHost->numSeg, a.segCap)) a.seg[i] = a.segHost[i];
+        if (i == 0) {
+            *a.dyn = *a.dynHost;
+            *a.errFlag = 0;
+        }
+        if (i < a.nbands) a.dynBands[i] = a.dynBandsHost[i];
     }
-    if (i < a.nbands) a.dynBands[i] = a.dynBandsHost[i];
     if (i < a.nZero) a.zeroWords[i] = 0u;
     if (a.tileFirst && i < a.ntiles) {
         a.tileFirst[i] = a.tileFirstInit;
diff --git a/planeverb_amd/csrc/pv_solver.cpp b/planeverb_amd/csrc/pv_solver.cpp
--- a/planeverb_amd/csrc/pv_solver.cpp
+++ b/planeverb_amd/csrc/pv_solver.cpp
@@ -334,6 +334,7 @@
             if (!dalloc(&nearBox_, 8, false)) return false;
             const int empty[8] = {INT_MAX, INT_MAX, -1, -1, INT_MAX, INT_MAX, -1, -1};
             if (!hipOk(hipMemcpyAsync(nearBox_, empty, sizeof(empty), hipMemcpyHostToDevice, stream_), "near box")) return false;
+            coverPrevKind_ = 1;
         }
     }
     scratchCount_ = std::max<size_t>({(size_t)3 * std::max(T_, g_.T), (size_t)lNX_ * g_.NY * 3,
@@ -1400,6 +1401,7 @@
     boundaryDirty_ = false;
     layerDirty_ = false;
     planesDirty_ = true;
+    coverPrevKind_ = 0;
     dynValid_ = false;
     dropGraph();
     tim_.geometryMs =
@@ -1595,8 +1597,10 @@
     return true;
 }
 
-void Solver::enqueueBeginRun(bool resetTiles) {
+void Solver::enqueueBeginRun(bool resetTiles, bool byValue) {
     BeginArgs b{};
+    b.byValue = byValue ? 1 : 0;
+    b.dynVal = dynCur_;
     b.dynHost = dynHost_;
     b.dyn = dynDev_;
     b.listHost = listHost_;
@@ -1752,7 +1756,7 @@
     plan_.oneXcd = xcdOk_ && (xcdWindowOk_ || probeWindow_) && blocks <= kResidentXcdMaxTiles &&
                    reserveBlocks(residentXcdInFlight(device_, xcdTarget_), blocks, kResidentXcdMaxTiles, &xcdHeld_);
     runTiles_ = blocks;
-    enqueueBeginRun(true);
+    enqueueBeginRun(true, true);
     launchResidentRun(12, win);
     for (int i = 0; i < 4; ++i) reachRect_[i] = win[i];
 }
@@ -2150,8 +2154,21 @@
 }
 
 void Solver::enqueueAnalysis(float lx, float lz) {
-    const AnalyzeArgs a = analyzeArgs(lx, lz);
+    AnalyzeArgs a = analyzeArgs(lx, lz);
     const bool carry = carryFrom_ && carryFrom_ != this && carryFrom_->device_ == device_ && !opt_.streaming && !isSlab();
+    lastCoverGroups_ = 0;
+    if (coverRun_ && a.box && !carry && opt_.analysisCover != 0) {
+        const int hist[4] = {dynCur_.histTileX0, dynCur_.histTileY0, dynCur_.histTilesX, dynCur_.histTilesY};
+        if (planAnalysisCover(runWin_, hist, rxi_, wi_, coverPrevKind_, coverPrevRect_, &a.cover)) lastCoverGroups_ = a.cover.groups;
+    }
+    coverPrevKind_ = 0;
+    if (coverRun_ && a.box) {
+        coverPrevKind_ = 2;
+        coverPrevRect_[0] = runWin_[0] * rxi_;
+        coverPrevRect_[1] = runWin_[2] * wi_;
+        coverPrevRect_[2] = runWin_[1] * rxi_;
+        coverPrevRect_[3] = runWin_[3] * wi_;
+    }
     if (carry) hipStreamWaitEvent(stream_, carryFrom_->ev_[2], 0);
     if (useFused_) {
         FusedArgs f{};
@@ -2200,6 +2217,8 @@
     if (pendingTimings_ && !sync()) return false;
     invalidateAnalysisMaps();
     lastRun_ = LastRun::Failed;
+    coverRun_ = false;
+    lastCoverGroups_ = 0;
     for (RecordSet& r : recs_) r.run = RecordSet::Run::None;
     if (!applyGeometry()) return false;
     PathRun r;
@@ -2219,6 +2238,7 @@
     launchCap_ = numGeneral_;
     if (kind == PathRun::Raw) {
         planesDirty_ = true;
+        coverPrevKind_ = 0;
         return true;
     }
     if (!zeroPlanesIfNeeded()) return false;
@@ -2245,7 +2265,11 @@
     if (plan_.reach && !clearReachPlanes(plan_.path == StepPath::Window && !repeating_ ? win : nullptr)) return false;
     if (!stampTimed()) hipEventRecord(ev_[0], stream_);
     switch (plan_.path) {
-        case StepPath::Window: enqueueWindowRun(win); break;
+        case StepPath::Window:
+            enqueueWindowRun(win);
+            coverRun_ = !probeWindow_ && !repeating_;
+            std::copy(win, win + 4, runWin_);
+            break;
         case StepPath::Resident: enqueueResidentRun(); break;
         case StepPath::SmallGrid:
             if (!enqueueSmallGridRun()) return false;
@@ -2934,6 +2958,7 @@
 bool Solver::setFields(const float* pr, const float* vx, const float* vy) {
     if (isSlab()) return fail("setFields is not available on a slab");
     planesDirty_ = true;
+    coverPrevKind_ = 0;
     if (!hipOk(hipSetDevice(device_), "hipSetDevice")) return false;
     const size_t n = (size_t)g_.NX * g_.NY;
     const float* src[3] = {pr, vx, vy};
diff --git a/planeverb_amd/csrc/pv_solver.h b/planeverb_amd/csrc/pv_solver.h
--- a/planeverb_amd/csrc/pv_solver.h
+++ b/planeverb_amd/csrc/pv_solver.h
@@ -50,6 +50,7 @@
     int rowBands = 0;
     int reachBound = -1;
     int residentWindow = -1;
+    int analysisCover = -1;
 };
 
 struct SolverTimings {
@@ -122,6 +123,7 @@
     const std::string& lastError() const { return err_; }
     bool streamFuse() const { return streamFuse_; }
     bool lastRunResidentWindow() const { return plan_.path == StepPath::Window; }
+    int lastRunAnalysisCover() const { return lastCoverGroups_; }
     bool lastRunOneXcd() const { return plan_.oneXcd; }
     bool residentKernel() const { return caps_.useResident && !layerActive(); }
     SolverOptions& options() { return opt_; }
@@ -302,7 +304,7 @@
     StepArgs baseStepArgs(bool withPulse, bool record) const;
     void setLaunchArgs(StepArgs& a, int t0, int k, bool firstOfRun, int li) const;
     bool prepareDyn(int lcx, int lcy, bool withPulse);
-    void enqueueBeginRun(bool resetTiles);
+    void enqueueBeginRun(bool resetTiles, bool byValue = false);
     bool zeroPlanesIfNeeded();
     AnalyzeArgs analyzeArgs(float lx, float lz) const;
     bool lazyFar_ = false;
@@ -316,6 +318,11 @@
     int nearPar_ = 0;
     bool useNearBox_ = false;
     bool nearBoxValid_ = false;
+    bool coverRun_ = false;
+    int runWin_[4] = {0, 0, 0, 0};
+    int coverPrevKind_ = 0;
+    int coverPrevRect_[4] = {0, 0, 0, 0};
+    int lastCoverGroups_ = 0;
     unsigned long long* stampsHost_ = nullptr;
     bool stampTimed() const { return (plan_.path == StepPath::Resident || plan_.path == StepPath::Window) && stampsHost_; }
     bool labelsValid_ = false;
```
